# klebgenomics/Kaptive

Hardware: AMD Instinct MI355X
Metric: assemblies typed/sec (K+O) (higher is better)
Workload: dtype uint16x2 (exact; int32-equivalent); 1 GPU; 10000 synthetic 5 Mbp kpsc assemblies per GPU typed against the synthetic K-locus database, then the O-locus database; one step = all of them, as 10 batches of 1000 through context-owned work buffers; packed assemblies resident in HBM before the timed region; one alignment pass over the genes of both databases, one reduction per database; alignment_passes_per_batch=1, assemblies_per_gpu=10000, assemblies_total=10000, batch=1000, parallelism=1 x independent shard, no collective

## Files before the change

kaptive_amd/csrc/kp_align.hip:

```cpp
#include "kp_host.h"

static const char *const NO_RESULTS = "this batch has no resident alignment results (not aligned yet, or displaced: a context keeps the results of its KP_WORK_SLOTS most recently aligned batches)";

static int enqueue_forked(kp_ctx *ctx, kp_batch *b, KpWork *w, hipStream_t stream) {
    const KpAnchors an = w->anchors();
    const KpTasks tasks = w->tasks();
    const KpJoins joins = w->joins();
    const KpTrace trace = w->trace();
    kp_launch_join_chain(an, tasks, w->groups(), joins, w->d_jscratch.p, ctx->opt.join, w->jstream);
    kp_launch_join_fill(b->view, ctx->genes, joins, trace, ctx->opt.join, w->jstream);
    kp_launch_join_trace(b->view, ctx->genes, joins, tasks, trace, ctx->opt.join, w->jstream);
    kp_launch_task_order(b->view, ctx->genes, an, tasks, stream);
    KP_HIP_CHECK(ctx, hipEventRecord(w->ev[KP_EV_ORDER], stream));
    kp_launch_sw(b->view, ctx->genes, tasks, trace, ctx->max_gene_len > KP_FILL16_MAX_GENE_LEN, stream, w->ev[KP_EV_FILL]);
    KP_HIP_CHECK(ctx, hipEventRecord(w->ev[KP_EV_TRACEBACK], stream));
    return KP_OK;
}

static int enqueue_align(kp_ctx *ctx, kp_batch *b, KpWork *w) {
    const size_t n_asm = w->n_asm;
    for (auto &e : w->ev)
        if (!e) KP_HIP_CHECK(ctx, hipEventCreate(&e.h));
    if (!w->astream) KP_HIP_CHECK(ctx, hipStreamCreateWithFlags(&w->astream.h, hipStreamNonBlocking));
    if (!w->jstream) {
        KP_HIP_CHECK(ctx, hipStreamCreateWithFlags(&w->jstream.h, hipStreamNonBlocking));
        KP_HIP_CHECK(ctx, hipEventCreateWithFlags(&w->ev_jfork.h, hipEventDisableTiming));
        KP_HIP_CHECK(ctx, hipEventCreateWithFlags(&w->ev_jdone.h, hipEventDisableTiming));
    }
    hipStream_t stream = w->astream;
    const Event *ev = w->ev;
    if ((uint64_t)n_asm * w->anchor_cap > 0xFFFFFFF0ull)
        return kp_fail(ctx, KP_EOVERFLOW, "anchor buffer would exceed 2^32 entries; use smaller batches");
    if (((uint64_t)b->view.total_words << 4) >> KP_CAND_POS_BITS)
        return kp_fail(ctx, KP_EOVERFLOW, "a batch holds at most 2^33 bases (candidate positions); use smaller batches");
    KP_HIP_CHECK(ctx, w->d_anchors_a.reserve(n_asm * w->anchor_cap));
    KP_HIP_CHECK(ctx, w->d_anchors_b.reserve(n_asm * w->anchor_cap));
    KP_HIP_CHECK(ctx, w->d_counts.reserve(w->counts_len()));
    KP_HIP_CHECK(ctx, w->d_sub_counts.reserve(n_asm * KP_ANCHOR_SUBS));
    KP_HIP_CHECK(ctx, w->d_seg.reserve(w->seg_len()));
    KP_HIP_CHECK(ctx, w->d_tasks.reserve(KP_N_CLASSES * (size_t)w->task_cap));
    KP_HIP_CHECK(ctx, w->d_results.reserve(KP_N_CLASSES * (size_t)w->task_cap));
    KP_HIP_CHECK(ctx, w->d_task_drop.reserve(KP_N_CLASSES * (size_t)w->task_cap));
    KP_HIP_CHECK(ctx, w->d_jscratch.reserve(kp_join_chain_scratch_bytes(ctx->opt.join)));
    {
        uint32_t lg = 12;
        while (((uint64_t)1 << lg) < (uint64_t)b->max_asm_bases * 2 / 5 + 1 && lg < 31) ++lg;
        w->occ_log2 = lg;
        KP_HIP_CHECK(ctx, w->d_occ_keys.reserve((size_t)w->occ_slots << lg));
        KP_HIP_CHECK(ctx, w->d_occ_cnts.reserve((size_t)w->occ_slots << lg));
        KP_HIP_CHECK(ctx, w->d_occ_state.reserve(kp_occ_state_words(n_asm, w->occ_slots)));
    }
    KP_HIP_CHECK(ctx, w->d_task_order.reserve(w->order_len()));
    KP_HIP_CHECK(ctx, w->d_cand.reserve(w->cand_cap));
    KP_HIP_CHECK(ctx, w->d_cand_count.reserve(KP_CAND_COUNTS));
    KP_HIP_CHECK(ctx, w->d_ends.reserve(KP_N_CLASSES * (size_t)w->task_cap));
    KP_HIP_CHECK(ctx, w->d_trace_top.reserve(KP_TOP_WORDS));
    KP_HIP_CHECK(ctx, w->d_trace.reserve(w->trace_cap));
    KP_HIP_CHECK(ctx, w->d_groups.reserve(w->group_cap));
    KP_HIP_CHECK(ctx, w->d_joins.reserve(KP_N_CLASSES * (size_t)w->join_cap));
    KP_HIP_CHECK(ctx, w->d_join_counts.reserve(KP_JOIN_COUNTS));
    KP_HIP_CHECK(ctx, hipStreamWaitEvent(stream, b->in->ready, 0));
    if (b->after && b->after->in) KP_HIP_CHECK(ctx, hipStreamWaitEvent(stream, b->after->in->ready, 0));
    KP_HIP_CHECK(ctx, hipMemsetAsync(w->d_counts.p, 0, w->counts_len() * sizeof(uint32_t), stream));
    KP_HIP_CHECK(ctx, hipMemsetAsync(w->d_sub_counts.p, 0, n_asm * KP_ANCHOR_SUBS * sizeof(uint32_t), stream));
    KP_HIP_CHECK(ctx, hipMemsetAsync(w->d_cand_count.p, 0, KP_CAND_COUNTS * sizeof(unsigned long long), stream));
    KP_HIP_CHECK(ctx, hipMemsetAsync(w->d_task_order.p, 0, KP_ORDER_HEAD * sizeof(uint32_t), stream));
    KP_HIP_CHECK(ctx, hipMemsetAsync(w->d_trace_top.p, 0, KP_TOP_WORDS * sizeof(unsigned long long), stream));
    KP_HIP_CHECK(ctx, hipMemsetAsync(w->d_join_counts.p, 0, KP_JOIN_COUNTS * sizeof(uint32_t), stream));
    auto bits_for = [](uint64_t max_value) { uint32_t n = 1; while (n < 63 && (max_value >> n)) ++n; return n; };
    w->key_bits.qb = std::min<uint32_t>(16, bits_for((uint64_t)std::max(ctx->max_gene_len, 1)));
    w->key_bits.db = std::min<uint32_t>(30, bits_for((uint64_t)b->max_asm_bases + KP_DIAG_BIAS));
    const KpAnchors an = w->anchors();
    KP_HIP_CHECK(ctx, hipEventRecord(ev[KP_EV_START], stream));
    kp_launch_scan(b->view, ctx->index, w->d_cand.p, w->d_cand_count.p, w->cand_cap, an, ctx->opt.scan_mode, b->n_ctg_total, stream, ev[KP_EV_SCAN]);
    if (!ctx->opt.library_sort && kp_bsort_fits(2u * (uint32_t)ctx->n_genes)) {
        kp_launch_anchor_bsort(b->view, an, 2u * (uint32_t)ctx->n_genes, stream);
    } else {
        kp_launch_anchor_compact(b->view, an, stream);
        int rc = kp_sort_anchors(ctx, an, b->n_asm, &w->sort_temp.p, &w->sort_temp.bytes, w->seg_begin(), w->seg_end(),
                                 (int)(w->key_bits.qb + w->key_bits.db) + ctx->gs_bits, stream);
        if (rc) return rc;
    }
    KP_HIP_CHECK(ctx, hipEventRecord(ev[KP_EV_SORT], stream));
    kp_launch_occ_cut(b->view, ctx->d_gene_len.p, an, w->d_occ_keys.p, w->d_occ_cnts.p, w->d_occ_state.p, w->occ_demand(), w->occ_slots, w->occ_log2, stream);
    kp_launch_chain(b->view, an, w->tasks(), w->groups(), stream);
    KP_HIP_CHECK(ctx, hipMemsetAsync(w->d_task_drop.p, 0, KP_N_CLASSES * (size_t)w->task_cap, stream));
    KP_HIP_CHECK(ctx, hipEventRecord(w->ev_jfork, stream));
    KP_HIP_CHECK(ctx, hipStreamWaitEvent(w->jstream, w->ev_jfork, 0));
    const int rc = enqueue_forked(ctx, b, w, stream);
    const hipError_t e_done = hipEventRecord(w->ev_jdone, w->jstream), e_join = hipStreamWaitEvent(stream, w->ev_jdone, 0);
    if (rc) return rc;
    KP_HIP_CHECK(ctx, e_done);
    KP_HIP_CHECK(ctx, e_join);
    KP_HIP_CHECK(ctx, hipEventRecord(ev[KP_EV_JOINED], stream));
    KP_HIP_CHECK(ctx, hipEventRecord(ev[KP_EV_END], stream));
    KP_HIP_CHECK(ctx, hipGetLastError());
    return KP_OK;
}

static int sync_runs(kp_ctx *ctx, KpWork *w) {
    KP_HIP_CHECK(ctx, hipStreamSynchronize(ctx->post));
    for (auto &r : w->runs)
        if (r && r->stream) { KP_HIP_CHECK(ctx, hipStreamSynchronize(r->stream)); if (r->aux) KP_HIP_CHECK(ctx, hipStreamSynchronize(r->aux)); }
    return KP_OK;
}

KpWork *finalised_work(kp_ctx *ctx, kp_batch *b) {
    KpWork *w = work_of(b);
    if (!w) { kp_fail(ctx, KP_ESTATE, NO_RESULTS); return nullptr; }
    if (!w->finalised) { kp_fail(ctx, KP_ESTATE, "kp_batch_wait has not completed"); return nullptr; }
    return w;
}

extern "C" {

int kp_batch_align(kp_ctx *ctx, kp_batch *b) {
    if (!ctx || !b || b->ctx != ctx) return kp_fail(ctx, KP_EINVAL, "bad context/batch");
    if (!ctx->has_db) return kp_fail(ctx, KP_ESTATE, "no database loaded");
    KP_HIP_CHECK(ctx, hipSetDevice(ctx->device));
    KpWork *w = work_of(b);
    if (!w) {
        w = &ctx->work[ctx->next_slot++ % KP_WORK_SLOTS];
        if (w->owner) {
            if (int rc = sync_runs(ctx, w)) return rc;
            w->owner->w = nullptr;
        }
        w->owner = b; w->n_asm = (size_t)b->n_asm;
        b->w = w; b->last_w = w;
    }
    kp_caps_size(ctx->opt, ctx->learnt, b->n_asm, b->view.total_words, *w);
    w->aligned = false; w->finalised = false;
    w->cs_on = ctx->opt.cs != 0; w->cs_valid = false;
    w->cigar_on = ctx->opt.cigar != 0 || w->cs_on; w->cigar_valid = false;
    for (auto &v : w->h_tasks) v.clear();
    w->reset_runs();
    w->stats[KP_STAT_RERUNS] = 0;
    int rc = enqueue_align(ctx, b, w);
    if (rc) return rc;
    w->aligned = true;
    return KP_OK;
}

static int finalise_hits_on_device(kp_ctx *ctx, kp_batch *b, KpWork *w) {
    const size_t n_asm = w->n_asm;
    for (int attempt = 0;; ++attempt) {
        KP_HIP_CHECK(ctx, w->d_hits_raw.reserve(n_asm * w->hit_cap));
        KP_HIP_CHECK(ctx, w->d_hits.reserve(n_asm * w->hit_cap));
        KP_HIP_CHECK(ctx, w->d_keys.reserve(n_asm * w->hit_cap * 3));
        KP_HIP_CHECK(ctx, w->d_hit_counts.reserve(w->hit_counts_len()));
        KP_HIP_CHECK(ctx, w->d_cells.reserve(1));
        KP_HIP_CHECK(ctx, hipMemsetAsync(w->d_hit_counts.p, 0, w->hit_counts_len() * sizeof(uint32_t), ctx->post));
        KP_HIP_CHECK(ctx, hipMemsetAsync(w->d_cells.p, 0, sizeof(unsigned long long), ctx->post));
        kp_launch_hit_finalise(b->view, ctx->d_gene_len.p, w->tasks(), w->joins(), w->raw_hits(), w->hits(), w->d_cells.p, ctx->ln_half(), ctx->ln_int(), ctx->post);
        KP_HIP_CHECK(ctx, hipGetLastError());
        w->h_hit_counts.resize(w->hit_counts_len());
        unsigned long long cells = 0;
        if (int frc = fetch_all(ctx, ctx->post, {{w->h_hit_counts.data(), w->d_hit_counts.p, w->hit_counts_len() * sizeof(uint32_t)}, {&cells, w->d_cells.p, sizeof cells}}))
            return frc;
        const uint32_t max_raw = n_asm ? *std::max_element(w->h_raw_hit_count(), w->h_raw_hit_count() + n_asm) : 0;
        if (max_raw <= w->hit_cap) { w->stats[KP_STAT_CELLS] = (int64_t)cells; break; }
        if (attempt >= 2) return kp_fail(ctx, KP_EOVERFLOW, "hit buffers overflowed repeatedly");
        kp_caps_grow_hits(ctx->learnt, *w, max_raw, true);
        w->stats[KP_STAT_RERUNS] += 1;
    }
    w->hit_off.assign(n_asm + 1, 0);
    for (size_t a = 0; a < n_asm; ++a) w->hit_off[a + 1] = w->hit_off[a] + (int64_t)w->h_hit_count()[a];
    return KP_OK;
}

static int emit_cigars(kp_ctx *ctx, kp_batch *b, KpWork *w) {
    const size_t n_asm = w->n_asm;
    const int64_t total = w->hit_off[n_asm];
    w->cigar_cap = kp_caps_cigar_size(ctx->opt, ctx->learnt, (uint64_t)total);
    KP_HIP_CHECK(ctx, w->d_cig_src.reserve(n_asm * w->hit_cap));
    KP_HIP_CHECK(ctx, w->d_cig_cnt.reserve((size_t)total));
    KP_HIP_CHECK(ctx, w->d_cig_off.reserve((size_t)total + 1));
    KP_HIP_CHECK(ctx, w->d_cig_hit_off.reserve(n_asm + 1));
    KP_HIP_CHECK(ctx, w->d_cig_ops.reserve(w->cigar_cap));
    KP_HIP_CHECK(ctx, hipMemcpyAsync(w->d_cig_hit_off.p, w->hit_off.data(), (n_asm + 1) * sizeof(int64_t), hipMemcpyHostToDevice, ctx->post));
    kp_launch_cigar_locate(b->view, ctx->d_gene_len.p, w->tasks(), w->joins(), w->hits(), w->d_cig_src.p, ctx->post);
    kp_launch_cigar_walk(b->view, ctx->genes, w->tasks(), w->joins(), w->trace(), w->hits(), w->hit_rows(), w->d_cig_src.p, w->cigars(), false, ctx->post);
    for (int attempt = 0;; ++attempt) {
        kp_launch_cigar_walk(b->view, ctx->genes, w->tasks(), w->joins(), w->trace(), w->hits(), w->hit_rows(), w->d_cig_src.p, w->cigars(), true, ctx->post);
        KP_HIP_CHECK(ctx, hipGetLastError());
        int64_t need = 0;
        if (int frc = fetch_all(ctx, ctx->post, {{&need, w->d_cig_off.p + total, sizeof need}})) return frc;
        w->cigar_total = need;
        if (kp_caps_after_cigar(ctx->learnt, w->cigar_cap, (uint64_t)total, (uint64_t)need)) break;
        if (attempt >= 1) return kp_fail(ctx, KP_EOVERFLOW, "CIGAR buffer overflowed repeatedly");
        KP_HIP_CHECK(ctx, w->d_cig_ops.reserve(w->cigar_cap));
    }
    w->cigar_valid = true;
    return KP_OK;
}

static int emit_cs(kp_ctx *ctx, kp_batch *b, KpWork *w) {
    const int64_t total = w->hit_off[w->n_asm];
    w->cs_cap = kp_caps_cs_size(ctx->cs_caps, (uint64_t)total);
    KP_HIP_CHECK(ctx, w->d_cs_cnt.reserve((size_t)total));
    KP_HIP_CHECK(ctx, w->d_cs_off.reserve((size_t)total + 1));
    KP_HIP_CHECK(ctx, w->d_cs_bytes.reserve(w->cs_cap));
    kp_launch_cs_walk(b->view, ctx->genes, w->hits(), w->hit_rows(), w->cigars(), w->cs(), false, ctx->post);
    for (int attempt = 0;; ++attempt) {
        kp_launch_cs_walk(b->view, ctx->genes, w->hits(), w->hit_rows(), w->cigars(), w->cs(), true, ctx->post);
        KP_HIP_CHECK(ctx, hipGetLastError());
        int64_t need = 0;
        if (int frc = fetch_all(ctx, ctx->post, {{&need, w->d_cs_off.p + total, sizeof need}})) return frc;
        w->cs_total = need;
        if (kp_caps_after_cs(ctx->cs_caps, w->cs_cap, (uint64_t)total, (uint64_t)need)) break;
        if (attempt >= 1) return kp_fail(ctx, KP_EOVERFLOW, "cs buffer overflowed repeatedly");
        KP_HIP_CHECK(ctx, w->d_cs_bytes.reserve(w->cs_cap));
    }
    w->cs_valid = true;
    return KP_OK;
}

static const char *const NO_CS = "this batch has no cs strings (aligned without the cs option, or its hit table was replaced)";
static const char *const NO_CIGARS = "this batch has no CIGARs (aligned without the cigar option, or its hit table was replaced)";

int kp_batch_wait(kp_ctx *ctx, kp_batch *b) {
    if (!ctx || !b || b->ctx != ctx) return kp_fail(ctx, KP_EINVAL, "bad context/batch");
    KpWork *w = work_of(b);
    if (!w || !w->aligned) return kp_fail(ctx, KP_ESTATE, w ? "kp_batch_align has not been called" : NO_RESULTS);
    if (w->finalised) return KP_OK;
    KP_HIP_CHECK(ctx, hipSetDevice(ctx->device));
    const size_t n_asm = w->n_asm;
    const uint32_t *const n_join = w->h_join_count();
    for (;;) {
        KP_HIP_CHECK(ctx, hipStreamWaitEvent(ctx->post, w->ev[KP_EV_END], 0));
        w->h_counts.resize(w->counts_len());
        unsigned long long n_cand[KP_CAND_COUNTS] = {}, top[KP_TOP_WORDS] = {};
        if (int frc = fetch_all(ctx, ctx->post, {{w->h_counts.data(), w->d_counts.p, w->counts_len() * sizeof(uint32_t)},
                                                 {n_cand, w->d_cand_count.p, sizeof n_cand}, {top, w->d_trace_top.p, sizeof top},
                                                 {w->h_join_counts, w->d_join_counts.p, sizeof w->h_join_counts}}))
            return frc;
        KpPassSeen seen;
        seen.n_asm = n_asm; seen.total_words = b->view.total_words; seen.n_cand = n_cand[KP_CAND_FRONT] + n_cand[KP_CAND_BACK];
        seen.trace_need = top[KP_TOP_TRACE]; seen.occ_need = top[KP_TOP_OCC];
        seen.n_group = w->h_group_count();
        for (int c = 0; c < KP_N_CLASSES; ++c) seen.max_join = std::max(seen.max_join, n_join[c]);
        for (size_t a = 0; a < n_asm; ++a) seen.max_slice = std::max(seen.max_slice, w->h_slice_need()[a]);
        for (int c = 0; c < KP_N_CLASSES; ++c) seen.max_task = std::max(seen.max_task, w->h_task_count()[c]);
        if (ctx->opt.join_stats)
            std::fprintf(stderr, "[kp_batch_wait] %zu assemblies: %u groups, joins per band class %u %u %u %u, %llu assemblies needed their mid_occ (%u tables)\n", n_asm, seen.n_group,
                         n_join[0], n_join[1], n_join[2], n_join[3], (unsigned long long)seen.occ_need, w->occ_slots);
        std::string err;
        const KpCapsVerdict verdict = kp_caps_after_pass(ctx->learnt, *w, seen, err);
        if (verdict == KP_CAPS_FITTED) break;
        if (verdict == KP_CAPS_OVERFLOW) return kp_fail(ctx, KP_EOVERFLOW, err);
        w->stats[KP_STAT_RERUNS] += 1;
        int rc = enqueue_align(ctx, b, w);
        if (rc) return rc;
    }
    int64_t n_anchor = 0, n_task = 0;
    for (size_t a = 0; a < n_asm; ++a) n_anchor += w->h_anchor_count()[a];
    for (int c = 0; c < KP_N_CLASSES; ++c) n_task += w->h_task_count()[c];
    for (auto &v : w->h_tasks) v.clear();
    w->h_joins.clear();
    int rc = finalise_hits_on_device(ctx, b, w);
    if (rc) return rc;
    w->stats[KP_STAT_ANCHORS] = n_anchor; w->stats[KP_STAT_TASKS] = n_task; w->stats[KP_STAT_HITS] = w->hit_off[n_asm];
    if (w->cigar_on)
        if (int crc = emit_cigars(ctx, b, w)) return crc;
    if (w->cs_on)
        if (int crc = emit_cs(ctx, b, w)) return crc;
    w->finalised = true;
    return KP_OK;
}

int kp_batch_hit_offsets(kp_ctx *ctx, kp_batch *b, int64_t *hit_off) {
    if (!ctx || !b || b->ctx != ctx || !hit_off) return kp_fail(ctx, KP_EINVAL, "bad arguments");
    KpWork *w = finalised_work(ctx, b);
    if (!w) return KP_ESTATE;
    std::memcpy(hit_off, w->hit_off.data(), w->hit_off.size() * sizeof(int64_t));
    return KP_OK;
}

int kp_batch_hits(kp_ctx *ctx, kp_batch *b, kp_hit *out, int64_t cap) {
    if (!ctx || !b || b->ctx != ctx || (!out && cap > 0)) return kp_fail(ctx, KP_EINVAL, "bad arguments");
    KpWork *w = finalised_work(ctx, b);
    if (!w) return KP_ESTATE;
    const size_t n_asm = w->n_asm;
    const KpHitTable hits = w->hits();
    if (cap < w->hit_off[n_asm]) return kp_fail(ctx, KP_EINVAL, "hit buffer too small");
    KP_HIP_CHECK(ctx, hipSetDevice(ctx->device));
    for (size_t a = 0; a < n_asm; ++a) {
        const int64_t n = w->hit_off[a + 1] - w->hit_off[a];
        if (n > 0)
            KP_HIP_CHECK(ctx, hipMemcpyAsync(out + w->hit_off[a], hits.of(a), (size_t)n * sizeof(kp_hit), hipMemcpyDeviceToHost, ctx->post));
    }
    KP_HIP_CHECK(ctx, hipStreamSynchronize(ctx->post));
    return KP_OK;
}

int kp_batch_set_hits(kp_ctx *ctx, kp_batch *b, const kp_hit *hits, const int64_t *hit_off) {
    if (!ctx || !b || b->ctx != ctx || !hit_off) return kp_fail(ctx, KP_EINVAL, "bad arguments");
    KpWork *w = finalised_work(ctx, b);
    if (!w) return KP_ESTATE;
    const size_t n_asm = w->n_asm;
    int64_t max_n = 0;
    for (size_t a = 0; a < n_asm; ++a) {
        const int64_t n = hit_off[a + 1] - hit_off[a];
        if (n < 0 || (n > 0 && !hits)) return kp_fail(ctx, KP_EINVAL, "hit offsets must ascend");
        max_n = std::max(max_n, n);
    }
    if (max_n > (1 << 24)) return kp_fail(ctx, KP_EOVERFLOW, "too many hits for one assembly");
    KP_HIP_CHECK(ctx, hipSetDevice(ctx->device));
    if (int rc = sync_runs(ctx, w)) return rc;
    if ((uint64_t)max_n > w->hit_cap) kp_caps_grow_hits(ctx->learnt, *w, (uint32_t)max_n, false);
    KP_HIP_CHECK(ctx, w->d_hits.reserve(n_asm * w->hit_cap));
    KP_HIP_CHECK(ctx, w->d_hit_counts.reserve(w->hit_counts_len()));
    w->h_hit_counts.resize(w->hit_counts_len());
    const KpHitTable table = w->hits();
    w->hit_off.assign(n_asm + 1, 0);
    for (size_t a = 0; a < n_asm; ++a) {
        const int64_t n = hit_off[a + 1] - hit_off[a];
        if (n > 0)
            KP_HIP_CHECK(ctx, hipMemcpy(table.of(a), hits + hit_off[a], (size_t)n * sizeof(kp_hit), hipMemcpyHostToDevice));
        w->h_hit_count()[a] = (uint32_t)n;
        w->hit_off[a + 1] = w->hit_off[a] + n;
    }
    if (n_asm)
        KP_HIP_CHECK(ctx, hipMemcpy(table.count, w->h_hit_count(), n_asm * sizeof(uint32_t), hipMemcpyHostToDevice));
    w->stats[KP_STAT_HITS] = w->hit_off[n_asm];
    w->cigar_valid = false; w->cs_valid = false;
    w->reset_runs();
    return KP_OK;
}

int kp_batch_cigar_offsets(kp_ctx *ctx, kp_batch *b, int64_t *cigar_off) {
    if (!ctx || !b || b->ctx != ctx || !cigar_off) return kp_fail(ctx, KP_EINVAL, "bad arguments");
    KpWork *w = finalised_work(ctx, b);
    if (!w) return KP_ESTATE;
    if (!w->cigar_valid) return kp_fail(ctx, KP_ESTATE, NO_CIGARS);
    KP_HIP_CHECK(ctx, hipSetDevice(ctx->device));
    KP_HIP_CHECK(ctx, hipMemcpyAsync(cigar_off, w->d_cig_off.p, ((size_t)w->hit_off[(size_t)b->n_asm] + 1) * sizeof(int64_t), hipMemcpyDeviceToHost, ctx->post));
    KP_HIP_CHECK(ctx, hipStreamSynchronize(ctx->post));
    return KP_OK;
}

int kp_batch_cigars(kp_ctx *ctx, kp_batch *b, uint32_t *ops, int64_t cap) {
    if (!ctx || !b || b->ctx != ctx || (!ops && cap > 0)) return kp_fail(ctx, KP_EINVAL, "bad arguments");
    KpWork *w = finalised_work(ctx, b);
    if (!w) return KP_ESTATE;
    if (!w->cigar_valid) return kp_fail(ctx, KP_ESTATE, NO_CIGARS);
    if (cap < w->cigar_total) return kp_fail(ctx, KP_EINVAL, "CIGAR buffer too small");
    KP_HIP_CHECK(ctx, hipSetDevice(ctx->device));
    if (w->cigar_total > 0) {
        KP_HIP_CHECK(ctx, hipMemcpyAsync(ops, w->d_cig_ops.p, (size_t)w->cigar_total * sizeof(uint32_t), hipMemcpyDeviceToHost, ctx->post));
        KP_HIP_CHECK(ctx, hipStreamSynchronize(ctx->post));
    }
    return KP_OK;
}

int kp_batch_cs_offsets(kp_ctx *ctx, kp_batch *b, int64_t *cs_off) {
    if (!ctx || !b || b->ctx != ctx || !cs_off) return kp_fail(ctx, KP_EINVAL, "bad arguments");
    KpWork *w = finalised_work(ctx, b);
    if (!w) return KP_ESTATE;
    if (!w->cs_valid) return kp_fail(ctx, KP_ESTATE, NO_CS);
    KP_HIP_CHECK(ctx, hipSetDevice(ctx->device));
    KP_HIP_CHECK(ctx, hipMemcpyAsync(cs_off, w->d_cs_off.p, ((size_t)w->hit_off[(size_t)b->n_asm] + 1) * sizeof(int64_t), hipMemcpyDeviceToHost, ctx->post));
    KP_HIP_CHECK(ctx, hipStreamSynchronize(ctx->post));
    return KP_OK;
}

int kp_batch_cs(kp_ctx *ctx, kp_batch *b, char *bytes, int64_t cap) {
    if (!ctx || !b || b->ctx != ctx || (!bytes && cap > 0)) return kp_fail(ctx, KP_EINVAL, "bad arguments");
    KpWork *w = finalised_work(ctx, b);
    if (!w) return KP_ESTATE;
    if (!w->cs_valid) return kp_fail(ctx, KP_ESTATE, NO_CS);
    if (cap < w->cs_total) return kp_fail(ctx, KP_EINVAL, "cs buffer too small");
    KP_HIP_CHECK(ctx, hipSetDevice(ctx->device));
    if (w->cs_total > 0) {
        KP_HIP_CHECK(ctx, hipMemcpyAsync(bytes, w->d_cs_bytes.p, (size_t)w->cs_total, hipMemcpyDeviceToHost, ctx->post));
        KP_HIP_CHECK(ctx, hipStreamSynchronize(ctx->post));
    }
    return KP_OK;
}

int kp_batch_stats(kp_ctx *ctx, kp_batch *b, int64_t *stats5) {
    if (!ctx || !b || b->ctx != ctx || !stats5) return kp_fail(ctx, KP_EINVAL, "bad arguments");
    KpWork *w = finalised_work(ctx, b);
    if (!w) return KP_ESTATE;
    std::memcpy(stats5, w->stats, sizeof w->stats);
    return KP_OK;
}

int kp_batch_profile(kp_ctx *ctx, kp_batch *b, float *ms7, int64_t *bytes_scanned) {
    if (!ctx || !b || b->ctx != ctx || !ms7) return kp_fail(ctx, KP_EINVAL, "bad arguments");
    KpWork *w = finalised_work(ctx, b);
    if (!w) return KP_ESTATE;
    KP_HIP_CHECK(ctx, hipSetDevice(ctx->device));
    for (int i = KP_EV_START; i < KP_EV_END; ++i) {
        const KpPassEvent next = KpPassEvent(i + 1);
        if (hipEventElapsedTime(&ms7[i], w->ev[i], w->ev[next]) != hipSuccess) return kp_fail(ctx, KP_EHIP, "event timing failed");
    }
    if (bytes_scanned) *bytes_scanned = 4 * b->view.total_words;
    return KP_OK;
}

int64_t kp_batch_anchors(kp_ctx *ctx, kp_batch *b, int32_t a, uint64_t *out, int64_t cap) {
    if (!ctx || !b || b->ctx != ctx || a < 0 || a >= b->n_asm) return kp_fail(ctx, KP_EINVAL, "bad arguments");
    KpWork *w = finalised_work(ctx, b);
    if (!w) return KP_ESTATE;
    const int64_t n = w->h_anchor_count()[a];
    const int64_t m = std::min(n, cap);
    if (out && m > 0) {
        if (hipMemcpy(out, w->anchors().of((size_t)a), (size_t)m * sizeof(uint64_t), hipMemcpyDeviceToHost) != hipSuccess)
            return kp_fail(ctx, KP_EHIP, "D2H anchors failed");
        for (int64_t i = 0; i < m; ++i) out[i] = kp_key_unpack(out[i], w->key_bits);
    }
    return n;
}

int64_t kp_batch_tasks(kp_ctx *ctx, kp_batch *b, int32_t a, int32_t *out8, int64_t cap) {
    if (!ctx || !b || b->ctx != ctx || a < 0 || a >= b->n_asm) return kp_fail(ctx, KP_EINVAL, "bad arguments");
    KpWork *w = finalised_work(ctx, b);
    if (!w) return KP_ESTATE;
    for (int c = 0; c < KP_N_CLASSES; ++c) {
        const size_t nt = w->h_task_count()[c];
        if (w->h_tasks[c].size() == nt) continue;
        w->h_tasks[c].resize(nt);
        if (nt && hipMemcpy(w->h_tasks[c].data(), w->tasks().cls(c), nt * sizeof(KpTask), hipMemcpyDeviceToHost) != hipSuccess)
            return kp_fail(ctx, KP_EHIP, "D2H tasks failed");
    }
    int64_t n = 0;
    for (int c = 0; c < KP_N_CLASSES; ++c)
        for (const KpTask &t : w->h_tasks[c]) {
            if (t.asm_id != a || t.n_anchors == 0) continue;
            if (out8 && n < cap) {
                int32_t *o = out8 + 8 * n;
                o[0] = t.gs; o[1] = t.contig; o[2] = t.lo; o[3] = t.width; o[4] = t.n_anchors; o[5] = (int32_t)(t.qspan & 0xFFFFu); o[6] = (int32_t)(t.qspan >> 16); o[7] = t.chain_score;
            }
            ++n;
        }
    return n;
}

int64_t kp_batch_task_results(kp_ctx *ctx, kp_batch *b, int32_t a, int32_t *out7, int64_t cap) {
    if (!ctx || !b || b->ctx != ctx || a < 0 || a >= b->n_asm) return kp_fail(ctx, KP_EINVAL, "bad arguments");
    const int64_t n_tasks = kp_batch_tasks(ctx, b, a, nullptr, 0);
    if (n_tasks < 0) return n_tasks;
    KpWork *w = finalised_work(ctx, b);
    if (!w) return KP_ESTATE;
    int64_t n = 0;
    std::vector<KpSwResult> res;
    for (int c = 0; c < KP_N_CLASSES; ++c) {
        const size_t nt = w->h_tasks[c].size();
        res.resize(nt);
        if (nt && hipMemcpy(res.data(), w->tasks().cls_results(c), nt * sizeof(KpSwResult), hipMemcpyDeviceToHost) != hipSuccess)
            return kp_fail(ctx, KP_EHIP, "D2H task results failed");
        for (size_t i = 0; i < nt; ++i) {
            if (w->h_tasks[c][i].asm_id != a || w->h_tasks[c][i].n_anchors == 0) continue;
            if (out7 && n < cap) {
                const KpSwResult &r = res[i];
                int32_t *o = out7 + 7 * n;
                o[0] = r.score; o[1] = r.q_start; o[2] = r.q_end; o[3] = r.t_start; o[4] = r.t_end; o[5] = r.matches; o[6] = r.block_len;
            }
            ++n;
        }
    }
    return n;
}

int64_t kp_batch_joins(kp_ctx *ctx, kp_batch *b, int32_t a, int32_t *out, int64_t cap) {
    if (!ctx || !b || b->ctx != ctx || a < 0 || a >= b->n_asm) return kp_fail(ctx, KP_EINVAL, "bad arguments");
    KpWork *w = finalised_work(ctx, b);
    if (!w) return KP_ESTATE;
    size_t total = 0;
    for (int c = 0; c < KP_N_CLASSES; ++c) total += w->h_join_count()[c];
    if (w->h_joins.size() != total) {
        w->h_joins.resize(total);
        size_t at = 0;
        for (int c = 0; c < KP_N_CLASSES; ++c) {
            const size_t nj = w->h_join_count()[c];
            if (nj && hipMemcpy(w->h_joins.data() + at, w->joins().cls(c), nj * sizeof(KpJoin), hipMemcpyDeviceToHost) != hipSuccess)
                return kp_fail(ctx, KP_EHIP, "D2H joins failed");
            at += nj;
        }
    }
    int64_t n = 0;
    for (const KpJoin &J : w->h_joins) {
        if (J.asm_id != a) continue;
        if (out && n < cap) {
            int32_t *o = out + KP_JOIN_ROW_INTS * n;
            std::memset(o, 0, KP_JOIN_ROW_INTS * sizeof(int32_t));
            o[0] = J.gs; o[1] = J.contig; o[2] = J.n_pieces; o[3] = J.n_anchors; o[4] = J.chain_score; o[5] = J.width;
            for (int k = 0; k < J.n_pieces; ++k) {
                o[6 + k] = J.lo[k];
                int32_t *pr = o + 6 + KP_JOIN_MAX_PIECES + 11 * k;
                pr[0] = J.state[k]; pr[1] = J.visited[k];
                if (J.state[k] == 1) std::memcpy(pr + 2, J.res[k], 9 * sizeof(int32_t));
            }
        }
        ++n;
    }
    return n;
}

}
```

kaptive_amd/csrc/kp_cigar.hip:

```cpp
#include <algorithm>

#include "kp_hits.h"
#include "kp_internal.h"
#include "kp_reduce_core.h"
#include "kp_walk.h"

namespace {

constexpr unsigned long long SRC_NONE = ~0ull;
constexpr int LO_BIAS = 1 << 30;
constexpr int WALK_THREADS = 256;
constexpr int SCAN_THREADS = 1024;

__device__ __forceinline__ unsigned long long src_key(bool join, int lo, uint32_t ref) {
    return ((unsigned long long)(join ? 1u : 0u) << 63) | ((unsigned long long)(uint32_t)(lo + LO_BIAS) << 32) | ref;
}

__device__ __forceinline__ void claim(const kp_hit *h, int n, const kp_hit &mine, unsigned long long key, unsigned long long *src) {
    for (int i = kp_lower_bound_gene(h, n, mine.gene); i < n && h[i].gene == mine.gene; ++i) {
        if (!kp_same_span(h[i], mine)) continue;
        if (h[i].score == KP_HIT_SCORE(mine.score) && h[i].matches == mine.matches && h[i].block_len == mine.block_len && h[i].n_seeds == mine.n_seeds)
            atomicMin(&src[i], key);
        return;
    }
}

__global__ __launch_bounds__(256) void kp_cigar_locate_tasks_kernel(KpBatchView b, const int32_t *__restrict__ gene_len,
                                                                    const KpTask *__restrict__ tasks, const KpSwResult *__restrict__ results,
                                                                    const uint8_t *__restrict__ task_drop, const uint32_t *__restrict__ task_count,
                                                                    uint32_t task_cap, const kp_hit *__restrict__ hits,
                                                                    const uint32_t *__restrict__ n_hits, uint32_t hit_cap,
                                                                    unsigned long long *__restrict__ src) {
    const int cls = blockIdx.y;
    uint32_t n = task_count[cls];
    if (n > task_cap) n = task_cap;
    for (uint32_t i = blockIdx.x * blockDim.x + threadIdx.x; i < n; i += gridDim.x * blockDim.x) {
        const size_t at = (size_t)cls * task_cap + i;
        const KpTask t = tasks[at];
        kp_hit mine;
        if (!kp_task_hit(b, gene_len, t, results[at], task_drop[at] != 0, &mine)) continue;
        claim(hits + (size_t)t.asm_id * hit_cap, (int)min(n_hits[t.asm_id], hit_cap), mine, src_key(false, t.lo, KP_TASK_REF(cls, i)),
              src + (size_t)t.asm_id * hit_cap);
    }
}

__device__ __forceinline__ uint32_t join_ref(int cls, uint32_t ji, int k) { return ((uint32_t)cls << 28) | (ji << 3) | (uint32_t)k; }
static_assert(KP_JOIN_MAX_PIECES <= 8, "three bits of a join's reference name the piece");

__global__ __launch_bounds__(64) void kp_cigar_locate_joins_kernel(KpBatchView b, const int32_t *__restrict__ gene_len,
                                                                   const KpJoin *__restrict__ joins, const uint32_t *__restrict__ join_count,
                                                                   uint32_t join_cap, const kp_hit *__restrict__ hits,
                                                                   const uint32_t *__restrict__ n_hits, uint32_t hit_cap,
                                                                   unsigned long long *__restrict__ src) {
    const int cls = blockIdx.y;
    uint32_t n = join_count[cls];
    if (n > join_cap) n = join_cap;
    for (uint32_t i = blockIdx.x * blockDim.x + threadIdx.x; i < n; i += gridDim.x * blockDim.x) {
        const KpJoin &J = joins[(size_t)cls * join_cap + i];
        for (int k = 1; k < J.n_pieces; ++k) {
            kp_hit mine;
            if (!kp_join_piece_hit(b, gene_len, J, k, &mine)) continue;
            claim(hits + (size_t)J.asm_id * hit_cap, (int)min(n_hits[J.asm_id], hit_cap), mine, src_key(true, J.lo[k], join_ref(cls, i, k)),
                  src + (size_t)J.asm_id * hit_cap);
        }
    }
}

struct OpRuns {
    uint32_t *out;
    int64_t pos, cap;
    int op = -1;
    uint32_t len = 0, n = 0;
    __device__ __forceinline__ void flush() {
        if (op < 0) return;
        ++n;
        if (out) {
            --pos;
            if (pos >= 0 && pos < cap) out[pos] = (len << 4) | (uint32_t)op;
        }
    }
    __device__ __forceinline__ void run(int o, int k) {
        if (k <= 0) return;
        if (o == op) { len += (uint32_t)k; return; }
        flush();
        op = o; len = (uint32_t)k;
    }
};

template <bool EMIT>
__global__ __launch_bounds__(WALK_THREADS) void kp_cigar_walk_kernel(KpBatchView b, KpGenes genes, const KpTask *__restrict__ tasks,
                                                                     const KpSwEnd *__restrict__ ends, uint32_t task_cap,
                                                                     const KpJoin *__restrict__ joins, uint32_t join_cap,
                                                                     const uint4 *__restrict__ trace, const uint32_t *__restrict__ n_hits,
                                                                     uint32_t hit_cap, const int64_t *__restrict__ hit_off,
                                                                     const unsigned long long *__restrict__ src, uint32_t *__restrict__ cnt,
                                                                     const int64_t *__restrict__ off, uint32_t *__restrict__ ops, int64_t ops_cap) {
    for (int a = blockIdx.x; a < b.n_asm; a += gridDim.x) {
        const uint32_t n = min(n_hits[a], hit_cap);
        for (uint32_t i0 = 0; i0 < n; i0 += WALK_THREADS) {
            const uint32_t i = i0 + threadIdx.x;
            const bool have = i < n;
            const unsigned long long key = have ? src[(size_t)a * hit_cap + i] : SRC_NONE;
            const bool is_join = key != SRC_NONE && (key >> 63) != 0, is_task = key != SRC_NONE && !is_join;
            const uint32_t ref = (uint32_t)key;
            const int cls = is_task || is_join ? (int)(ref >> 28) : 0, P = 4 << cls;
            const int64_t row = hit_off[a] + i;
            OpRuns v;
            v.out = EMIT ? ops : nullptr; v.cap = ops_cap; v.pos = EMIT && have ? off[row + 1] : 0;
            KpTask tk;
            tk.asm_id = a; tk.gs = 0; tk.contig = 0; tk.lo = 0;
            KpSwEnd e;
            e.score = 0; e.er = 0; e.eb = 0; e.trace_off = 0;
            const KpJoin *J = joins + (size_t)cls * join_cap + (is_join ? (ref & 0x0FFFFFFFu) >> 3 : 0u);
            if (is_task) {
                const size_t at = (size_t)cls * task_cap + KP_REF_SLOT(ref);
                tk = tasks[at]; e = ends[at];
            }
            const KpTaskSeqs s = kp_task_seqs(b, genes, a, is_join ? J->gs : tk.gs, is_join ? J->contig : tk.contig);
            int q0 = 0, r_hi;
            if (is_task) kp_task_rows(tk.lo, 4 * P, s.t.cstart, s.t.cend, s.q.len, &q0, &r_hi);
            KpBandPath bp;
            kp_band_walk(is_task, tk.lo, P, q0, e.er, e.eb & 255, false, trace + e.trace_off, s, bp, v);
            if (is_join) {
                KpJoinPath jp;
                kp_join_walk(J, (int)(ref & 7u), P, s, trace, jp, v);
            }
            v.flush();
            if (!EMIT && have) cnt[row] = v.n;
        }
    }
}

__global__ __launch_bounds__(SCAN_THREADS) void kp_cigar_scan_kernel(const uint32_t *__restrict__ cnt, int64_t n, int64_t *__restrict__ off) {
    __shared__ int64_t s_sum[SCAN_THREADS];
    const int tid = threadIdx.x;
    const int64_t per = (n + SCAN_THREADS - 1) / SCAN_THREADS;
    const int64_t lo = (int64_t)tid * per < n ? (int64_t)tid * per : n, hi = lo + per < n ? lo + per : n;
    int64_t mine = 0;
    for (int64_t i = lo; i < hi; ++i) mine += cnt[i];
    s_sum[tid] = mine;
    __syncthreads();
    for (int o = 1; o < SCAN_THREADS; o <<= 1) {
        const int64_t v = tid >= o ? s_sum[tid - o] : 0;
        __syncthreads();
        s_sum[tid] += v;
        __syncthreads();
    }
    int64_t at = s_sum[tid] - mine;
    for (int64_t i = lo; i < hi; ++i) { off[i] = at; at += cnt[i]; }
    if (tid == SCAN_THREADS - 1) off[n] = s_sum[tid];
}

}

void kp_launch_cigar_locate(const KpBatchView &b, const int32_t *gene_len, const KpTasks &t, const KpJoins &j, const KpHitTable &hits,
                            unsigned long long *src, hipStream_t stream) {
    (void)hipMemsetAsync(src, 0xFF, (size_t)b.n_asm * hits.cap * sizeof(unsigned long long), stream);
    hipLaunchKernelGGL(kp_cigar_locate_tasks_kernel, dim3(256, KP_N_CLASSES), dim3(256), 0, stream, b, gene_len, t.tasks, t.results, t.drop, t.count,
                       t.cap, hits.rows, hits.count, hits.cap, src);
    hipLaunchKernelGGL(kp_cigar_locate_joins_kernel, dim3(16, KP_N_CLASSES), dim3(64), 0, stream, b, gene_len, j.list, j.count, j.cap, hits.rows,
                       hits.count, hits.cap, src);
}

void kp_launch_count_scan(const uint32_t *cnt, int64_t n, int64_t *off, hipStream_t stream) {
    hipLaunchKernelGGL(kp_cigar_scan_kernel, dim3(1), dim3(SCAN_THREADS), 0, stream, cnt, n, off);
}

void kp_launch_cigar_walk(const KpBatchView &b, const KpGenes &genes, const KpTasks &t, const KpJoins &j, const KpTrace &trace, const KpHitTable &hits,
                          const KpHitRows &rows, const unsigned long long *src, const KpPerHit<uint32_t> &cig, bool emit, hipStream_t stream) {
    const dim3 grid((unsigned)std::min(std::max(b.n_asm, 1), 4096)), block(WALK_THREADS);
    if (!emit) {
        hipLaunchKernelGGL(kp_cigar_walk_kernel<false>, grid, block, 0, stream, b, genes, t.tasks, t.ends, t.cap, j.list, j.cap, trace.units, hits.count,
                           hits.cap, rows.hit_off, src, cig.cnt, (const int64_t *)nullptr, (uint32_t *)nullptr, (int64_t)0);
        return kp_launch_count_scan(cig.cnt, rows.total, cig.off, stream);
    }
    hipLaunchKernelGGL(kp_cigar_walk_kernel<true>, grid, block, 0, stream, b, genes, t.tasks, t.ends, t.cap, j.list, j.cap, trace.units, hits.count,
                       hits.cap, rows.hit_off, src, (uint32_t *)nullptr, cig.off, cig.data, cig.cap);
}
```

kaptive_amd/csrc/kp_ctx.hip:

```cpp
#include <cctype>
#include <cstdlib>
#include <mutex>
#include <new>
#include <unordered_map>
#include <sys/mman.h>

#include "kp_host.h"

static std::mutex g_err_mutex;
static std::string g_global_error = "";

std::atomic<long long> g_dev_allocs{0};
bool g_debug_alloc = false;

static std::mutex g_pin_mutex;
struct PinBlock { size_t bytes; bool mapped, locked; };
static std::unordered_map<void *, PinBlock> g_pin_blocks;
static size_t g_pin_bytes = 0;
constexpr size_t HUGE_PAGE = (size_t)2 << 20;
hipError_t pinned_alloc(void **out, size_t bytes) {
    const hipError_t e = hipHostMalloc(out, bytes, hipHostMallocPortable);
    if (e == hipSuccess) {
        std::lock_guard<std::mutex> lk(g_pin_mutex);
        g_pin_blocks[*out] = PinBlock{bytes, false, true};
        g_pin_bytes += bytes;
    }
    return e;
}
static void *mapped_alloc(size_t bytes) {
    bytes = (bytes + HUGE_PAGE - 1) & ~(HUGE_PAGE - 1);
    char *raw = (char *)mmap(nullptr, bytes + HUGE_PAGE, PROT_READ | PROT_WRITE, MAP_PRIVATE | MAP_ANONYMOUS, -1, 0);
    if (raw == MAP_FAILED) return nullptr;
    char *p = (char *)(((uintptr_t)raw + HUGE_PAGE - 1) & ~(uintptr_t)(HUGE_PAGE - 1));
    if (p > raw) munmap(raw, (size_t)(p - raw));
    if (raw + HUGE_PAGE > p) munmap(p + bytes, (size_t)(raw + HUGE_PAGE - p));
    (void)madvise(p, bytes, MADV_HUGEPAGE);
    std::lock_guard<std::mutex> lk(g_pin_mutex);
    g_pin_blocks[p] = PinBlock{bytes, true, false};
    return p;
}
static hipError_t mapped_lock(void *p) {
    size_t bytes;
    {
        std::lock_guard<std::mutex> lk(g_pin_mutex);
        auto it = g_pin_blocks.find(p);
        if (it == g_pin_blocks.end() || !it->second.mapped) return hipErrorInvalidValue;
        if (it->second.locked) return hipSuccess;
        bytes = it->second.bytes;
    }
    const hipError_t e = hipHostRegister(p, bytes, hipHostRegisterPortable);
    if (e == hipSuccess) {
        std::lock_guard<std::mutex> lk(g_pin_mutex);
        g_pin_blocks[p].locked = true;
        g_pin_bytes += bytes;
    }
    return e;
}
void pinned_free(void *p) {
    if (!p) return;
    PinBlock b{0, false, true};
    {
        std::lock_guard<std::mutex> lk(g_pin_mutex);
        auto it = g_pin_blocks.find(p);
        if (it != g_pin_blocks.end()) {
            b = it->second;
            if (b.locked) g_pin_bytes -= b.bytes;
            g_pin_blocks.erase(it);
        }
    }
    if (b.mapped) {
        if (b.locked) (void)hipHostUnregister(p);
        munmap(p, b.bytes);
    } else {
        (void)hipHostFree(p);
    }
}

int kp_fail(kp_ctx *ctx, int code, const std::string &msg) {
    if (ctx) ctx->error = msg;
    else {
        std::lock_guard<std::mutex> lk(g_err_mutex);
        g_global_error = msg;
    }
    return code;
}

hipError_t create_priority_stream(hipStream_t *stream) {
    int least = 0, greatest = 0;
    hipError_t e = hipDeviceGetStreamPriorityRange(&least, &greatest);
    if (e != hipSuccess) return e;
    return hipStreamCreateWithPriority(stream, hipStreamDefault, greatest);
}

static uint32_t env_u32(const char *name, uint32_t dflt) {
    const char *v = std::getenv(name);
    if (!v || !*v) return dflt;
    const long long x = std::atoll(v);
    return x > 0 ? (uint32_t)x : dflt;
}

static void options_from_env(KpOptions &o) {
    o.anchor_cap = env_u32("KAPTIVE_AMD_ANCHOR_CAP", o.anchor_cap);
    o.tasks_per_asm = env_u32("KAPTIVE_AMD_TASKS_PER_ASM", o.tasks_per_asm);
    o.hit_cap = env_u32("KAPTIVE_AMD_HIT_CAP", o.hit_cap);
    o.trace_kb_per_asm = env_u32("KAPTIVE_AMD_TRACE_KB_PER_ASM", o.trace_kb_per_asm);
    o.trace_set = env_u32("KAPTIVE_AMD_TRACE_KB_PER_ASM", 0) != 0;
    o.cand_cap = env_u32("KAPTIVE_AMD_CAND_CAP", 0);
    o.group_cap = env_u32("KAPTIVE_AMD_GROUP_CAP", o.group_cap);
    o.join_cap = env_u32("KAPTIVE_AMD_JOIN_CAP", o.join_cap);
    o.occ_slots = env_u32("KAPTIVE_AMD_OCC_SLOTS", o.occ_slots);
    o.kept_cap = env_u32("KAPTIVE_AMD_KEPT_CAP", o.kept_cap);
    o.piece_cap = env_u32("KAPTIVE_AMD_PIECE_CAP", o.piece_cap);
    o.prot_cap = env_u32("KAPTIVE_AMD_PROT_CAP", o.prot_cap);
    o.scan_mode = (int)env_u32("KAPTIVE_AMD_SCAN_ABLATE", 0);
    o.library_sort = (int)env_u32("KAPTIVE_AMD_LIBRARY_SORT", 0);
    o.upload_piece_mb = std::max<uint32_t>(1, env_u32("KAPTIVE_AMD_UPLOAD_PIECE_MB", 4096));
    { const char *rb = getenv("KAPTIVE_AMD_READBACK"); o.readback_copy_engine = rb && std::string(rb) == "copy"; }
    o.spin_wait = (int)env_u32("KAPTIVE_AMD_SPIN_WAIT", 0);
    o.join_stats = std::getenv("KAPTIVE_AMD_JOIN_STATS") != nullptr;
    if (const char *e = std::getenv("KAPTIVE_AMD_JOIN_GRID")) std::sscanf(e, "%d,%d,%d,%d", &o.join.fill, &o.join.walk, &o.join.chain, &o.join.chain_large);
    if (const char *e = std::getenv("KAPTIVE_AMD_JOIN_PRIO")) o.join.prio = std::atoi(e);
    if (const char *e = std::getenv("KAPTIVE_AMD_SKIP_JOINS")) o.join.skip = std::atoi(e);
    g_debug_alloc = std::getenv("KAPTIVE_AMD_DEBUG_ALLOC") != nullptr;
}

static void fill_blosum(int8_t *m) {
    static const int8_t b[25][25] = {
        {4, -1, -2, -2, 0, -1, -1, 0, -2, -1, -1, -1, -1, -2, -1, 1, 0, -3, -2, 0, -2, -1, -1, -1, -4},
        {-1, 5, 0, -2, -3, 1, 0, -2, 0, -3, -2, 2, -1, -3, -2, -1, -1, -3, -2, -3, -1, -2, 0, -1, -4},
        {-2, 0, 6, 1, -3, 0, 0, 0, 1, -3, -3, 0, -2, -3, -2, 1, 0, -4, -2, -3, 4, -3, 0, -1, -4},
        {-2, -2, 1, 6, -3, 0, 2, -1, -1, -3, -4, -1, -3, -3, -1, 0, -1, -4, -3, -3, 4, -3, 1, -1, -4},
        {0, -3, -3, -3, 9, -3, -4, -3, -3, -1, -1, -3, -1, -2, -3, -1, -1, -2, -2, -1, -3, -1, -3, -1, -4},
        {-1, 1, 0, 0, -3, 5, 2, -2, 0, -3, -2, 1, 0, -3, -1, 0, -1, -2, -1, -2, 0, -2, 4, -1, -4},
        {-1, 0, 0, 2, -4, 2, 5, -2, 0, -3, -3, 1, -2, -3, -1, 0, -1, -3, -2, -2, 1, -3, 4, -1, -4},
        {0, -2, 0, -1, -3, -2, -2, 6, -2, -4, -4, -2, -3, -3, -2, 0, -2, -2, -3, -3, -1, -4, -2, -1, -4},
        {-2, 0, 1, -1, -3, 0, 0, -2, 8, -3, -3, -1, -2, -1, -2, -1, -2, -2, 2, -3, 0, -3, 0, -1, -4},
        {-1, -3, -3, -3, -1, -3, -3, -4, -3, 4, 2, -3, 1, 0, -3, -2, -1, -3, -1, 3, -3, 3, -3, -1, -4},
        {-1, -2, -3, -4, -1, -2, -3, -4, -3, 2, 4, -2, 2, 0, -3, -2, -1, -2, -1, 1, -4, 3, -3, -1, -4},
        {-1, 2, 0, -1, -3, 1, 1, -2, -1, -3, -2, 5, -1, -3, -1, 0, -1, -3, -2, -2, 0, -3, 1, -1, -4},
        {-1, -1, -2, -3, -1, 0, -2, -3, -2, 1, 2, -1, 5, 0, -2, -1, -1, -1, -1, 1, -3, 2, -1, -1, -4},
        {-2, -3, -3, -3, -2, -3, -3, -3, -1, 0, 0, -3, 0, 6, -4, -2, -2, 1, 3, -1, -3, 0, -3, -1, -4},
        {-1, -2, -2, -1, -3, -1, -1, -2, -2, -3, -3, -1, -2, -4, 7, -1, -1, -4, -3, -2, -2, -3, -1, -1, -4},
        {1, -1, 1, 0, -1, 0, 0, 0, -1, -2, -2, 0, -1, -2, -1, 4, 1, -3, -2, -2, 0, -2, 0, -1, -4},
        {0, -1, 0, -1, -1, -1, -1, -2, -2, -1, -1, -1, -1, -2, -1, 1, 5, -2, -2, 0, -1, -1, -1, -1, -4},
        {-3, -3, -4, -4, -2, -2, -3, -2, -2, -3, -2, -3, -1, 1, -4, -3, -2, 11, 2, -3, -4, -2, -2, -1, -4},
        {-2, -2, -2, -3, -2, -1, -2, -3, 2, -1, -1, -2, -1, 3, -3, -2, -2, 2, 7, -1, -3, -1, -2, -1, -4},
        {0, -3, -3, -3, -1, -2, -2, -3, -3, 3, 1, -2, 1, -1, -2, -2, 0, -3, -1, 4, -3, 2, -2, -1, -4},
        {-2, -1, 4, 4, -3, 0, 1, -1, 0, -3, -4, 0, -3, -3, -2, 0, -1, -4, -3, -3, 4, -3, 0, -1, -4},
        {-1, -2, -3, -3, -1, -2, -3, -4, -3, 3, 3, -3, 2, 0, -3, -2, -1, -2, -1, 2, -3, 3, -3, -1, -4},
        {-1, 0, 0, 1, -3, 4, 4, -2, 0, -3, -3, 1, -1, -3, -1, 0, -1, -2, -2, -2, 0, -3, 4, -1, -4},
        {-1, -1, -1, -1, -1, -1, -1, -1, -1, -1, -1, -1, -1, -1, -1, -1, -1, -1, -1, -1, -1, -1, -1, -1, -4},
        {-4, -4, -4, -4, -4, -4, -4, -4, -4, -4, -4, -4, -4, -4, -4, -4, -4, -4, -4, -4, -4, -4, -4, -4, 1},
    };
    static const char alphabet[] = "ARNDCQEGHILKMFPSTWYVBJZX*";
    std::memset(m, KP_PROT_FILL, 256 * 256);
    for (int x = 0; x < 25; ++x)
        for (int y = 0; y < 25; ++y) m[(uint8_t)alphabet[x] * 256 + (uint8_t)alphabet[y]] = b[x][y];
}

extern "C" {

int kp_device_count(void) {
    int n_dev = 0;
    const hipError_t e = hipGetDeviceCount(&n_dev);
    if (e != hipSuccess) return kp_fail(nullptr, KP_EHIP, std::string("hipGetDeviceCount: ") + hipGetErrorString(e));
    return n_dev;
}

int kp_device_numa_node(int device_id) {
    char bus[64] = {0};
    if (hipDeviceGetPCIBusId(bus, (int)sizeof bus, device_id) != hipSuccess) return -1;
    for (char *c = bus; *c; ++c) *c = (char)std::tolower((unsigned char)*c);
    const std::string path = std::string("/sys/bus/pci/devices/") + bus + "/numa_node";
    std::FILE *f = std::fopen(path.c_str(), "r");
    if (!f) return -1;
    int node = -1;
    if (std::fscanf(f, "%d", &node) != 1) node = -1;
    std::fclose(f);
    return node;
}

int kp_ctx_create(int device_id, kp_ctx **out) {
    if (!out) return kp_fail(nullptr, KP_EINVAL, "out is null");
    *out = nullptr;
    int n_dev = 0;
    hipError_t e = hipGetDeviceCount(&n_dev);
    if (e != hipSuccess || n_dev == 0)
        return kp_fail(nullptr, KP_EHIP, std::string("no HIP device available: ") + hipGetErrorString(e));
    if (device_id < 0 || device_id >= n_dev) return kp_fail(nullptr, KP_EINVAL, "device_id out of range");
    kp_ctx *ctx = new (std::nothrow) kp_ctx();
    if (!ctx) return kp_fail(nullptr, KP_ENOMEM, "out of host memory");
    ctx->device = device_id;
    options_from_env(ctx->opt);
    if ((e = hipSetDevice(device_id)) == hipSuccess && !ctx->opt.spin_wait) (void)hipSetDeviceFlags(hipDeviceScheduleBlockingSync);
    if (e != hipSuccess || (e = hipStreamCreate(&ctx->stream.h)) != hipSuccess || (e = hipStreamCreateWithFlags(&ctx->copy.h, hipStreamNonBlocking)) != hipSuccess ||
        (e = create_priority_stream(&ctx->post.h)) != hipSuccess || (e = create_priority_stream(&ctx->aux.h)) != hipSuccess) {
        delete ctx;
        return kp_fail(nullptr, KP_EHIP, std::string("device setup failed: ") + hipGetErrorString(e));
    }
    std::vector<int8_t> m(256 * 256);
    fill_blosum(m.data());
    std::vector<float> ln(KP_MAPQ_LN_HALF_SIZE + KP_MAPQ_LN_INT_SIZE, 0.0f);
    for (int i = 1; i < KP_MAPQ_LN_HALF_SIZE; ++i) ln[(size_t)i] = kp_mapq_ln((double)i / 2.0);
    for (int i = 1; i < KP_MAPQ_LN_INT_SIZE; ++i) ln[(size_t)KP_MAPQ_LN_HALF_SIZE + i] = kp_mapq_ln((double)i);
    if (upload(ctx, ctx->d_blosum, m.data(), m.size()) != KP_OK || upload(ctx, ctx->d_ln, ln.data(), ln.size()) != KP_OK || hipStreamSynchronize(ctx->stream) != hipSuccess) {
        std::string msg = ctx->error;
        kp_ctx_destroy(ctx);
        return kp_fail(nullptr, KP_EHIP, "substitution table upload failed: " + msg);
    }
    *out = ctx;
    return KP_OK;
}

void kp_ctx_destroy(kp_ctx *ctx) {
    if (!ctx) return;
    (void)hipSetDevice(ctx->device);
    (void)hipDeviceSynchronize();
    for (kp_batch *b : ctx->batches) {
        b->in.reset();
        b->ctx = nullptr; b->w = nullptr; b->last_w = nullptr;
    }
    delete ctx;
}

const char *kp_last_error(const kp_ctx *ctx) {
    if (ctx) return ctx->error.c_str();
    std::lock_guard<std::mutex> lk(g_err_mutex);
    static thread_local std::string copy;
    copy = g_global_error;
    return copy.c_str();
}

void *kp_ctx_stream(kp_ctx *ctx) { return ctx ? (void *)ctx->stream.h : nullptr; }

int kp_ctx_set_option(kp_ctx *ctx, const char *name, int64_t value) {
    if (!ctx) return kp_fail(nullptr, KP_EINVAL, "null context");
    if (!name || value < 0) return kp_fail(ctx, KP_EINVAL, "bad option");
    const std::string n(name);
    KpOptions &o = ctx->opt;
    if (kp_caps_set_option(o, ctx->learnt, ctx->run_caps, n, value)) return KP_OK;
    if (kp_caps_set_cs_option(ctx->cs_caps, n, value)) return KP_OK;
    if (n == "scan_mode") o.scan_mode = (int)value;
    else if (n == "library_sort") o.library_sort = value != 0;
    else if (n == "cigar") o.cigar = value != 0;
    else if (n == "cs") o.cs = value != 0;
    else if (n == "upload_piece_mb") o.upload_piece_mb = (uint32_t)std::max<int64_t>(1, std::min<int64_t>(value, 4096));
    else return kp_fail(ctx, KP_EINVAL, "unknown option: " + n);
    return KP_OK;
}

int kp_host_alloc(size_t bytes, void **out) {
    if (!out) return kp_fail(nullptr, KP_EINVAL, "out is null");
    *out = nullptr;
    if (bytes >= 4 * HUGE_PAGE) {
        int rc = kp_host_reserve(bytes, out);
        if (rc == KP_OK && (rc = kp_host_lock(*out)) == KP_OK) return KP_OK;
        if (*out) { pinned_free(*out); *out = nullptr; }
    }
    const hipError_t e = pinned_alloc(out, std::max<size_t>(bytes, 1));
    if (e != hipSuccess) return kp_fail(nullptr, KP_ENOMEM, std::string("hipHostMalloc: ") + hipGetErrorString(e));
    return KP_OK;
}

int kp_host_reserve(size_t bytes, void **out) {
    if (!out) return kp_fail(nullptr, KP_EINVAL, "out is null");
    *out = mapped_alloc(std::max<size_t>(bytes, 1));
    if (!*out) return kp_fail(nullptr, KP_ENOMEM, "mmap failed");
    return KP_OK;
}

int kp_host_lock(void *p) {
    const hipError_t e = mapped_lock(p);
    if (e == hipErrorInvalidValue) return kp_fail(nullptr, KP_EINVAL, "not a block of kp_host_reserve");
    if (e != hipSuccess) return kp_fail(nullptr, KP_ENOMEM, std::string("hipHostRegister: ") + hipGetErrorString(e));
    return KP_OK;
}

void kp_host_free(void *p) { pinned_free(p); }

int64_t kp_device_allocations(void) { return (int64_t)g_dev_allocs.load(std::memory_order_relaxed); }

int64_t kp_host_pinned_bytes(void) {
    std::lock_guard<std::mutex> lk(g_pin_mutex);
    return (int64_t)g_pin_bytes;
}

}
```

kaptive_amd/csrc/kp_host.h:

```cpp
#pragma once

#include <cstring>
#include <memory>
#include "kp_internal.h"
#include "kp_caps.h"
#include "kp_device.h"
#include "kp_reduce_core.h"
static_assert(KP_CAPS_ANCHOR_SUBS == KP_ANCHOR_SUBS, "the policy sizes the scan's sub-slices");

struct KpTypingGroup {
    int32_t gene_lo = 0, gene_hi = 0;
    DevBuf<uint16_t> d_gene_locus, d_gene_pos;
    DevBuf<uint8_t> d_gene_extra, d_prot_db;
    DevBuf<int8_t> d_gene_strand;
    DevBuf<int32_t> d_locus_off, d_locus_len, d_prot_db_off, d_prot_db_len;
    KpTypingDb typing{};
    int max_db_prot_len = 0;
};

struct KpTypingRun {
    hipStream_t stream = nullptr, aux = nullptr;
    Event ev_fork, ev_join;
    bool split = false;
    KpHitTable hits{};
    DevBuf<kp_hit> d_hits;
    DevBuf<uint32_t> d_hit_n;
    DevBuf<uint64_t> d_keys;
    DevBuf<uint32_t> d_order;
    DevBuf<uint8_t> d_flag;
    DevBuf<int32_t> d_dp_scratch;
    int kept_cap = 0, piece_cap = 0, prot_cap = 0;
    size_t n_asm = 0;
    DevBuf<uint32_t> d_pack;
    DevBuf<uint8_t> d_prot;
    DevBuf<double> d_scores;
    DevBuf<int32_t> d_lcounts, d_best, d_pairs, d_dp;
    DevBuf<KpKept> d_kept;
    DevBuf<KpPiece> d_pieces;
    DevBuf<KpAsmSummary> d_summary;
    KpTypingParams prm{};
    bool scored = false, reduced = false;
    bool sums_valid = false;
    std::vector<KpAsmSummary> h_sums;
    int32_t max_kept = 1, max_pieces = 1;
    size_t slots() const { return n_asm * (size_t)kept_cap; }
    size_t pairs_len() const { return 4 * slots() + n_asm + 1; }
    KpReduceTables tables() const {
        int32_t *const q = d_pairs.p, *const base = q + 4 * slots();
        return {.best = d_best.p, .keys = d_keys.p, .order = d_order.p, .kept_flag = d_flag.p, .kept = d_kept.p, .kept_cap = kept_cap,
                .pieces = d_pieces.p, .piece_cap = piece_cap, .summary = d_summary.p, .prot = d_prot.p, .prot_cap = prot_cap,
                .q_off = q, .q_len = q + slots(), .t_off = q + 2 * slots(), .t_len = q + 3 * slots(), .pair_base = base, .n_pairs = base + n_asm, .dp8 = d_dp.p};
    }
};

struct kp_batch;

struct KpOptions : KpCapOptions {
    int scan_mode = 0;
    int library_sort = 0;
    uint32_t upload_piece_mb = 4096;
    int readback_copy_engine = 0;
    int spin_wait = 0;
    int cigar = 0;
    int cs = 0;
    bool join_stats = false;
    KpJoinLaunch join;
};

struct KpInput {
    DevBuf<uint32_t> d_words;
    DevBuf<int64_t> d_asm_word_off;
    DevBuf<int32_t> d_ctg_start, d_ctg_len, d_asm_first_ctg, d_n_runs, d_asm_first_nrun;
    PinnedBlock h_stage;
    Event ready;
};

enum KpPassEvent { KP_EV_START, KP_EV_SCAN, KP_EV_SORT, KP_EV_ORDER, KP_EV_FILL, KP_EV_TRACEBACK, KP_EV_JOINED, KP_EV_END, KP_N_EVENTS };
static_assert(KP_EV_END == 7, "kp_batch_profile returns seven stage times");
enum KpStat { KP_STAT_ANCHORS, KP_STAT_TASKS, KP_STAT_CELLS, KP_STAT_HITS, KP_STAT_RERUNS, KP_N_STATS };
enum KpTopWord { KP_TOP_TRACE = 0, KP_TOP_OCC = 3, KP_TOP_WORDS = 4 };
enum KpJoinCount { KP_JOIN_GROUPS = 0, KP_JOIN_CLASSES = 1, KP_JOIN_COUNTS = 1 + KP_N_CLASSES };
enum KpCandCount { KP_CAND_FRONT, KP_CAND_BACK, KP_CAND_COUNTS };

struct KpWork : KpPassCaps {
    kp_batch *owner = nullptr;
    size_t n_asm = 0;
    KpKeyBits key_bits{16, 30};
    DevBuf<uint64_t> d_anchors_a, d_anchors_b;
    DevBuf<uint32_t> d_counts;
    size_t task_count_at() const { return n_asm; }
    size_t slice_need_at() const { return n_asm + KP_N_CLASSES; }
    size_t counts_len() const { return slice_need_at() + n_asm; }
    const uint32_t *h_anchor_count() const { return h_counts.data(); }
    const uint32_t *h_task_count() const { return h_counts.data() + task_count_at(); }
    const uint32_t *h_slice_need() const { return h_counts.data() + slice_need_at(); }
    DevBuf<uint32_t> d_sub_counts;
    DevBuf<uint64_t> d_cand;
    DevBuf<unsigned long long> d_cand_count;
    DevBuf<uint32_t> d_seg;
    size_t seg_len() const { return 2 * n_asm; }
    uint32_t *seg_begin() const { return d_seg.p; }
    uint32_t *seg_end() const { return d_seg.p + n_asm; }
    DevBuf<KpTask> d_tasks;
    DevBuf<KpSwResult> d_results;
    DevBuf<uint8_t> d_task_drop, d_jscratch;
    DevBuf<uint32_t> d_occ_keys, d_occ_cnts, d_occ_state;
    uint32_t occ_log2 = 0;
    DevBuf<KpSwEnd> d_ends;
    DevBuf<unsigned long long> d_trace_top;
    unsigned long long *occ_demand() const { return d_trace_top.p + KP_TOP_OCC; }
    Stream astream;
    Stream jstream;
    Event ev_jfork, ev_jdone;
    DevBuf<uint4> d_trace;
    DevBlock sort_temp;
    DevBuf<uint32_t> d_task_order;
    size_t order_len() const { return KP_ORDER_HEAD + KP_N_CLASSES * (size_t)task_cap; }
    DevBuf<KpGroup> d_groups;
    DevBuf<KpJoin> d_joins;
    DevBuf<uint32_t> d_join_counts;
    uint32_t h_join_counts[KP_JOIN_COUNTS] = {};
    uint32_t h_group_count() const { return h_join_counts[KP_JOIN_GROUPS]; }
    const uint32_t *h_join_count() const { return h_join_counts + KP_JOIN_CLASSES; }
    std::vector<KpJoin> h_joins;
    DevBuf<kp_hit> d_hits_raw, d_hits;
    DevBuf<uint32_t> d_hit_counts;
    size_t hit_counts_len() const { return 2 * n_asm; }
    uint32_t *h_raw_hit_count() { return h_hit_counts.data(); }
    uint32_t *h_hit_count() { return h_hit_counts.data() + n_asm; }
    DevBuf<uint64_t> d_keys;
    DevBuf<unsigned long long> d_cells;
    bool cigar_on = false, cigar_valid = false;
    uint64_t cigar_cap = 0;
    int64_t cigar_total = 0;
    DevBuf<unsigned long long> d_cig_src;
    DevBuf<uint32_t> d_cig_cnt, d_cig_ops;
    DevBuf<int64_t> d_cig_off, d_cig_hit_off;
    bool cs_on = false, cs_valid = false;
    uint64_t cs_cap = 0;
    int64_t cs_total = 0;
    DevBuf<uint32_t> d_cs_cnt;
    DevBuf<int64_t> d_cs_off;
    DevBuf<char> d_cs_bytes;
    std::vector<std::unique_ptr<KpTypingRun>> runs;
    bool aligned = false, finalised = false;
    std::vector<uint32_t> h_counts, h_hit_counts;
    std::vector<KpTask> h_tasks[KP_N_CLASSES];
    std::vector<int64_t> hit_off;
    int64_t stats[KP_N_STATS] = {};
    Event ev[KP_N_EVENTS];
    KpAnchors anchors() const {
        return {.keys = d_anchors_a.p, .count = d_counts.p, .cap = anchor_cap, .kb = key_bits, .sub_count = d_sub_counts.p,
                .sub_cap = anchor_cap / KP_ANCHOR_SUBS, .second = d_anchors_b.p, .need = d_counts.p + slice_need_at()};
    }
    KpTasks tasks() const {
        return {.tasks = d_tasks.p, .count = d_counts.p + task_count_at(), .cap = task_cap, .results = d_results.p, .ends = d_ends.p, .drop = d_task_drop.p,
                .order_head = d_task_order.p, .order_count = d_task_order.p + KP_ORDER_COUNTS, .order = d_task_order.p + KP_ORDER_HEAD};
    }
    KpGroups groups() const { return {.list = d_groups.p, .count = d_join_counts.p + KP_JOIN_GROUPS, .cap = group_cap}; }
    KpJoins joins() const { return {.list = d_joins.p, .count = d_join_counts.p + KP_JOIN_CLASSES, .cap = join_cap}; }
    KpTrace trace() const { return {.units = d_trace.p, .top = d_trace_top.p + KP_TOP_TRACE, .cap = trace_cap}; }
    KpHitTable raw_hits() const { return {.rows = d_hits_raw.p, .count = d_hit_counts.p, .cap = hit_cap, .keys = d_keys.p}; }
    KpHitTable hits() const { return {.rows = d_hits.p, .count = d_hit_counts.p + n_asm, .cap = hit_cap, .keys = nullptr}; }
    KpHitRows hit_rows() const { return {.hit_off = d_cig_hit_off.p, .total = hit_off[n_asm]}; }
    KpPerHit<uint32_t> cigars() const { return {.cnt = d_cig_cnt.p, .off = d_cig_off.p, .data = d_cig_ops.p, .cap = (int64_t)cigar_cap}; }
    KpPerHit<char> cs() const { return {.cnt = d_cs_cnt.p, .off = d_cs_off.p, .data = d_cs_bytes.p, .cap = (int64_t)cs_cap}; }
    void reset_runs() { for (auto &r : runs) if (r) r->split = r->scored = r->reduced = r->sums_valid = false; }
};

#define KP_INPUT_POOL 16

struct kp_ctx {
    int device = 0;
    PinnedBlock bounce;
    int gs_bits = 18;
    int max_gene_len = 0;
    Stream stream;
    Stream post;
    Stream aux;
    Stream copy;
    std::string error;
    KpOptions opt;
    KpLearnt learnt;
    KpCsCaps cs_caps;
    bool has_db = false;
    int32_t n_genes = 0;
    int64_t n_postings = 0;
    std::vector<int32_t> gene_len;
    DevBuf<uint2> d_slots;
    DevBuf<uint64_t> d_filter, d_filter2;
    DevBuf<uint64_t> d_postings;
    DevBuf<uint32_t> d_nib;
    DevBuf<int32_t> d_nib_off, d_gene_len;
    DevBuf<uint4> d_gene_prof;
    DevBuf<uint8_t> d_gene_has_n;
    KpSeedIndex index{};
    KpGenes genes{};
    DevBuf<int8_t> d_blosum;
    DevBuf<float> d_ln;
    const float *ln_half() const { return d_ln.p; }
    const float *ln_int() const { return d_ln.p + KP_MAPQ_LN_HALF_SIZE; }
    DevBuf<uint8_t> d_pq, d_pt;
    DevBuf<int32_t> d_pmeta, d_pout, d_pscratch;
    std::vector<std::unique_ptr<KpTypingGroup>> groups;
    std::vector<KpRunCaps> run_caps;
    struct GroupStreams { Stream stream, aux; };
    std::vector<GroupStreams> group_streams;
    KpWork work[KP_WORK_SLOTS];
    uint32_t next_slot = 0;
    std::vector<std::unique_ptr<KpInput>> free_inputs;
    std::vector<kp_batch *> batches;
};

struct kp_batch {
    kp_ctx *ctx = nullptr;
    int32_t n_asm = 0;
    std::unique_ptr<KpInput> in;
    const uint32_t *d_words = nullptr;
    KpBatchView view{};
    int64_t max_asm_bases = 0;
    int32_t n_ctg_total = 0;
    KpWork *w = nullptr;
    KpWork *last_w = nullptr;
    kp_batch *after = nullptr;
    int32_t group = 0;
};

hipError_t create_priority_stream(hipStream_t *stream);

struct Fetch {
    kp_ctx *ctx;
    hipStream_t stream;
    struct Item { void *dst; size_t off, bytes; };
    std::vector<Item> items;
    size_t used = 0;
    bool by_copy_engine;
    Fetch(kp_ctx *c, hipStream_t s) : ctx(c), stream(s), by_copy_engine(c->opt.readback_copy_engine != 0) {}
    ~Fetch() { if (!items.empty()) (void)hipStreamSynchronize(stream); }
    int begin(size_t total) {
        if (by_copy_engine) return KP_OK;
        total += 64 * 8;
        KP_HIP_CHECK(ctx, ctx->bounce.reserve(total, total + total / 4 + (1u << 20)));
        return KP_OK;
    }
    int add(void *dst, const void *src, size_t bytes) {
        if (!bytes) return KP_OK;
        if (by_copy_engine || (bytes & 3u)) { KP_HIP_CHECK(ctx, hipMemcpyAsync(dst, src, bytes, hipMemcpyDeviceToHost, stream)); return KP_OK; }
        if (used + bytes > ctx->bounce.bytes) return kp_fail(ctx, KP_ESTATE, "read-back larger than announced");
        kp_launch_read_back(src, ctx->bounce.p + used, bytes, stream);
        items.push_back(Item{dst, used, bytes});
        used = (used + bytes + 63) & ~(size_t)63;
        return KP_OK;
    }
    int finish() {
        const hipError_t e = hipStreamSynchronize(stream);
        if (e != hipSuccess) { items.clear(); used = 0; }
        KP_HIP_CHECK(ctx, e);
        for (const Item &it : items) std::memcpy(it.dst, ctx->bounce.p + it.off, it.bytes);
        items.clear(); used = 0;
        return KP_OK;
    }
};

struct FetchItem { void *dst; const void *src; size_t bytes; };
inline int fetch_all(kp_ctx *ctx, hipStream_t stream, std::initializer_list<FetchItem> items) {
    size_t total = 0;
    for (const FetchItem &i : items) total += i.bytes;
    Fetch f(ctx, stream);
    int rc = f.begin(total);
    for (const FetchItem &i : items) if (!rc) rc = f.add(i.dst, i.src, i.bytes);
    return rc ? rc : f.finish();
}

template <class T>
int upload(kp_ctx *ctx, DevBuf<T> &buf, const T *src, size_t n, hipStream_t stream = nullptr) {
    KP_HIP_CHECK(ctx, buf.reserve(n));
    if (n) KP_HIP_CHECK(ctx, hipMemcpyAsync(buf.p, src, n * sizeof(T), hipMemcpyHostToDevice, stream ? stream : ctx->stream.h));
    return KP_OK;
}

inline KpWork *work_of(kp_batch *b) {
    return (b->w && b->w->owner == b) ? b->w : nullptr;
}
KpWork *finalised_work(kp_ctx *ctx, kp_batch *b);
```

kaptive_amd/csrc/kp_internal.h:

```cpp
#pragma once

#include <hip/hip_runtime.h>
#include <stdint.h>

#include <string>
#include <vector>

#include "../../include/kaptive_amd.h"

#define KP_FILTER_LOG2 24
__host__ __device__ inline uint32_t kp_filter_block(uint32_t x) { return x & ((1u << (KP_FILTER_LOG2 - 6)) - 1u); }
__host__ __device__ inline uint2 kp_filter_mask2(uint32_t x) {
    uint2 m;
    m.x = 1u << ((x >> 18) & 31u);
    m.y = 1u << ((x >> 23) & 31u);
    return m;
}
__host__ __device__ inline bool kp_filter_test(uint2 got, uint32_t x) {
    return ((got.x >> ((x >> 18) & 31u)) & (got.y >> ((x >> 23) & 31u)) & 1u) != 0u;
}
__host__ __device__ inline uint64_t kp_filter_mask(uint32_t kmer) {
    const uint2 m = kp_filter_mask2(kmer);
    return ((uint64_t)m.y << 32) | m.x;
}
#define KP_FILTER2_LOG2 23
__host__ __device__ inline uint32_t kp_filter2_block(uint32_t kmer) { return (kmer * 0xC2B2AE35u) >> (32 - (KP_FILTER2_LOG2 - 6)); }
__host__ __device__ inline uint2 kp_filter2_mask2(uint32_t kmer) {
    const uint32_t h = kmer * 0x27D4EB2Fu;
    uint2 m;
    m.x = (1u << (h >> 27)) | (1u << ((h >> 22) & 31u));
    m.y = (1u << ((h >> 17) & 31u)) | (1u << ((h >> 12) & 31u));
    return m;
}
#define KP_CAND_POS_BITS 33
__host__ __device__ inline uint64_t kp_cand_pack(uint64_t pos, uint32_t z, uint32_t x) { return (pos << 31) | ((uint64_t)z << 30) | x; }
__host__ __device__ inline bool kp_seed_is_interior(int64_t t, int64_t S, int64_t E) { return t >= S + KP_W && t + KP_K + KP_W <= E; }

struct KpSeedIndex {
    const uint64_t *filter;
    const uint64_t *filter2;
    const uint2 *slots;
    const uint64_t *postings;
    uint32_t slot_mask;
    uint32_t slot_shift;
};

struct KpGenes {
    const uint32_t *nib;
    const int32_t *word_off;
    const int32_t *len;
    int32_t n_genes;
    const uint4 *prof;
    const uint8_t *has_n;
};

__host__ __device__ inline uint32_t kp_row_profile(uint32_t qcode) {
    return qcode < 4u ? ((6u << (3u * qcode)) | (3u << 12)) : (3u | (3u << 3) | (3u << 6) | (3u << 9) | (3u << 12));
}

struct KpKeyBits {
    uint32_t qb, db;
};
__host__ __device__ inline uint64_t kp_key_pack(uint64_t spec_key, KpKeyBits kb) {
    return ((spec_key >> 46) << (kb.qb + kb.db)) | (((spec_key >> 16) & 0x3FFFFFFFull) << kb.qb) | (spec_key & 0xFFFFull);
}
__host__ __device__ inline uint32_t kp_ckey_qpos(uint64_t k, KpKeyBits kb) { return (uint32_t)(k & ((1ull << kb.qb) - 1ull)); }
__host__ __device__ inline uint32_t kp_ckey_diag(uint64_t k, KpKeyBits kb) {
    return (uint32_t)((k >> kb.qb) & ((1ull << kb.db) - 1ull));
}
__host__ __device__ inline uint32_t kp_ckey_gs(uint64_t k, KpKeyBits kb) { return (uint32_t)(k >> (kb.qb + kb.db)); }
__host__ __device__ inline uint64_t kp_key_unpack(uint64_t k, KpKeyBits kb) {
    return ((uint64_t)kp_ckey_gs(k, kb) << 46) | ((uint64_t)kp_ckey_diag(k, kb) << 16) | kp_ckey_qpos(k, kb);
}

struct KpBatchView {
    const uint32_t *words;
    const int64_t *asm_word_off;
    const int32_t *ctg_start;
    const int32_t *ctg_len;
    const int32_t *asm_first_ctg;
    const int32_t *n_runs;
    const int32_t *asm_first_nrun;
    int32_t n_asm;
    int64_t total_words;
};

#define KP_N_CLASSES 4
struct KpTask {
    int32_t asm_id;
    int32_t gs;
    int32_t contig;
    int32_t lo;
    int32_t width;
    int32_t n_anchors;
    uint32_t qspan;
    int32_t chain_score;
};
static_assert(sizeof(KpTask) == 32, "KpTask is read as two 16-byte halves");

struct KpSwResult {
    int32_t score, q_start, q_end, t_start, t_end, matches, block_len;
};

__host__ __device__ inline void kp_task_rows(int lo, int width, int cstart, int cend, int qlen, int *r_lo, int *r_hi);
__host__ __device__ inline void kp_piece_rows(int lo, int width, int cstart, int cend, int qlen, int r0, int r1, int *r_lo, int *r_hi) {
    kp_task_rows(lo, width, cstart, cend, qlen, r_lo, r_hi);
    if (*r_lo < r0) *r_lo = r0;
    if (*r_hi > r1) *r_hi = r1;
    if (*r_hi < *r_lo) *r_hi = *r_lo;
}
__host__ __device__ inline void kp_task_rows(int lo, int width, int cstart, int cend, int qlen, int *r_lo, int *r_hi) {
    int a = cstart - lo - (width - 1);
    if (a < 0) a = 0;
    a &= ~7;
    int z = cend - lo;
    if (z > qlen) z = qlen;
    if (z < a) z = a;
    *r_lo = a;
    *r_hi = z;
}

struct KpSwEnd {
    int32_t score;
    int32_t er, eb;
    uint32_t trace_off;
};
#define KP_SWEND_HAS_N 0x100

#define KP_TASK_REF(cls, slot) (((uint32_t)(cls) << 28) | (uint32_t)(slot))
#define KP_REF_CLS(ref) ((ref) >> 28)
#define KP_REF_SLOT(ref) ((ref) & 0x0FFFFFFFu)
#define KP_REF_NONE 0xFFFFFFFFu
struct KpGroup {
    int32_t asm_id, n;
    int32_t gs, contig;
    uint32_t total;
    uint32_t task[KP_JOIN_GROUP_MAX];
    uint32_t first[KP_JOIN_GROUP_MAX];
    uint32_t cnt[KP_JOIN_GROUP_MAX];
};
struct KpJoin {
    int32_t asm_id, gs, contig, n_pieces, n_anchors, chain_score, width;
    int32_t lo[KP_JOIN_MAX_PIECES];
    int32_t cmask[KP_JOIN_MAX_PIECES];
    int32_t r0[KP_JOIN_MAX_PIECES], r1[KP_JOIN_MAX_PIECES];
    int32_t n_members;
    int32_t weak_mask;
    uint32_t member_task[KP_JOIN_GROUP_MAX];
    uint32_t trace_off[KP_JOIN_MAX_PIECES], export_off[KP_JOIN_MAX_PIECES];
    int32_t end_s[KP_JOIN_MAX_PIECES], end_r[KP_JOIN_MAX_PIECES], end_b[KP_JOIN_MAX_PIECES];
    int32_t state[KP_JOIN_MAX_PIECES], visited[KP_JOIN_MAX_PIECES];
    int32_t res[KP_JOIN_MAX_PIECES][9];
    int32_t drop_mask;
};

#define KP_HIP_CHECK(ctx, expr)                                                                     \
    do {                                                                                            \
        hipError_t e_ = (expr);                                                                     \
        if (e_ != hipSuccess) return kp_fail((ctx), KP_EHIP, std::string(#expr) + ": " + hipGetErrorString(e_)); \
    } while (0)

struct kp_ctx;
int kp_fail(kp_ctx *ctx, int code, const std::string &msg);

struct KpAnchors {
    uint64_t *keys;
    uint32_t *count;
    uint32_t cap;
    KpKeyBits kb;
    uint32_t *sub_count;
    uint32_t sub_cap;
    uint64_t *second;
    uint32_t *need;
    uint64_t *of(size_t a) const { return keys + a * cap; }
};
struct KpTasks {
    KpTask *tasks;
    uint32_t *count;
    uint32_t cap;
    KpSwResult *results;
    KpSwEnd *ends;
    uint8_t *drop;
    uint32_t *order_head, *order_count, *order;
    KpTask *cls(int c) const { return tasks + (size_t)c * cap; }
    KpSwResult *cls_results(int c) const { return results + (size_t)c * cap; }
};
struct KpGroups { KpGroup *list; uint32_t *count; uint32_t cap; };
struct KpJoins { KpJoin *list; uint32_t *count ; uint32_t cap; KpJoin *cls(int c) const { return list + (size_t)c * cap; } };
struct KpTrace { uint4 *units; unsigned long long *top; uint64_t cap; };
struct KpHitTable {
    kp_hit *rows;
    uint32_t *count;
    uint32_t cap;
    uint64_t *keys;
    kp_hit *of(size_t a) const { return rows + a * cap; }
};
struct KpHitRows { const int64_t *hit_off; int64_t total; };
template <class T>
struct KpPerHit { uint32_t *cnt; int64_t *off; T *data; int64_t cap; };
struct KpReduceTables {
    const int32_t *best;
    uint64_t *keys;
    uint32_t *order;
    uint8_t *kept_flag;
    kp_kept *kept; int kept_cap;
    kp_piece *pieces; int piece_cap;
    kp_asm_summary *summary;
    uint8_t *prot; int prot_cap;
    int32_t *q_off, *q_len, *t_off, *t_len, *pair_base, *n_pairs;
    int32_t *dp8;
};
struct KpJoinLaunch { int fill = 2048, walk = 512, chain = 2560, chain_large = 512, prio = 1, skip = 0; };

#define KP_ANCHOR_SUBS 64
void kp_launch_scan(const KpBatchView &b, const KpSeedIndex &idx, uint64_t *cand, unsigned long long *n_cand, uint64_t cand_cap,
                    const KpAnchors &an, int ablate_mode, int32_t n_ctg_total, hipStream_t stream, hipEvent_t after_scan);
void kp_launch_anchor_compact(const KpBatchView &b, const KpAnchors &an, hipStream_t stream);
size_t kp_occ_state_words(size_t n_asm, uint32_t occ_slots);
void kp_launch_occ_cut(const KpBatchView &b, const int32_t *gene_len, const KpAnchors &an, uint32_t *occ_keys, uint32_t *occ_cnts,
                       uint32_t *occ_state, unsigned long long *occ_demand, uint32_t occ_slots, uint32_t occ_log2_size, hipStream_t stream);
void kp_launch_chain(const KpBatchView &b, const KpAnchors &an, const KpTasks &tasks, const KpGroups &groups, hipStream_t stream);
void kp_launch_sw(const KpBatchView &b, const KpGenes &genes, const KpTasks &tasks, const KpTrace &trace, bool has_long_genes, hipStream_t stream, hipEvent_t after_fill);
#define KP_ORDER_BUCKETS 65
#define KP_ORDER_COUNTS (2 * KP_N_CLASSES * KP_ORDER_BUCKETS)
#define KP_ORDER_HEAD (KP_ORDER_COUNTS + 2 * KP_N_CLASSES)
void kp_launch_task_order(const KpBatchView &b, const KpGenes &genes, const KpAnchors &an, const KpTasks &tasks, hipStream_t stream);
void kp_launch_join_chain(const KpAnchors &an, const KpTasks &tasks, const KpGroups &groups, const KpJoins &joins, uint8_t *scratch,
                          const KpJoinLaunch &L, hipStream_t stream);
size_t kp_join_chain_scratch_bytes(const KpJoinLaunch &L);
void kp_launch_join_fill(const KpBatchView &b, const KpGenes &genes, const KpJoins &joins, const KpTrace &trace, const KpJoinLaunch &L, hipStream_t stream);
void kp_launch_join_trace(const KpBatchView &b, const KpGenes &genes, const KpJoins &joins, const KpTasks &tasks, const KpTrace &trace,
                          const KpJoinLaunch &L, hipStream_t stream);
void kp_launch_cigar_locate(const KpBatchView &b, const int32_t *gene_len, const KpTasks &tasks, const KpJoins &joins, const KpHitTable &hits,
                            unsigned long long *src, hipStream_t stream);
void kp_launch_cigar_walk(const KpBatchView &b, const KpGenes &genes, const KpTasks &tasks, const KpJoins &joins, const KpTrace &trace, const KpHitTable &hits,
                          const KpHitRows &rows, const unsigned long long *src, const KpPerHit<uint32_t> &cig, bool emit, hipStream_t stream);
void kp_launch_count_scan(const uint32_t *cnt, int64_t n, int64_t *off, hipStream_t stream);
void kp_launch_cs_walk(const KpBatchView &b, const KpGenes &genes, const KpHitTable &hits, const KpHitRows &rows, const KpPerHit<uint32_t> &cig,
                       const KpPerHit<char> &cs, bool emit, hipStream_t stream);
void kp_launch_hit_split(const KpHitTable &hits, int32_t gene_lo, int32_t gene_hi, const KpHitTable &out, int32_t n_asm, hipStream_t stream);
struct KpTypingDb;
void kp_launch_hit_finalise(const KpBatchView &b, const int32_t *gene_len, const KpTasks &tasks, const KpJoins &joins, const KpHitTable &raw,
                            const KpHitTable &hits, unsigned long long *cells, const float *ln_half, const float *ln_int, hipStream_t stream);
void kp_launch_score(const KpBatchView &b, const KpHitTable &hits, const KpTypingDb &db, double min_cov, double *scores, int32_t *counts, hipStream_t stream);
void kp_launch_reduce(const KpBatchView &b, const KpHitTable &hits, const KpTypingDb &db, const kp_typing_params &prm, const KpReduceTables &t, hipStream_t stream);
void kp_launch_states(const KpBatchView &b, const KpTypingDb &db, const kp_typing_params &prm, const KpReduceTables &t, hipStream_t stream);
void kp_launch_read_back(const void *src, void *dst_pinned, size_t bytes, hipStream_t stream);
void kp_launch_pack_rows(const uint32_t *src, size_t src_pitch, uint32_t *dst, size_t dst_pitch, size_t width, int rows,
                         hipStream_t stream);
#define KP_PROT_ROWBUF_FIELDS 8
void kp_launch_protein(const uint8_t *q, const int32_t *q_off, const int32_t *q_len, const uint8_t *t,
                       const int32_t *t_off, const int32_t *t_len, int32_t n, const int32_t *n_dev, const int8_t *blosum,
                       int32_t *out8, int32_t *scratch, size_t scratch_ints_per_block, int n_blocks, hipStream_t stream,
                       hipStream_t aux, hipEvent_t fork, hipEvent_t join,
                       const int32_t *seed_off = nullptr, int seed_k = 0);
bool kp_bsort_fits(uint32_t n_bins);
void kp_launch_anchor_bsort(const KpBatchView &b, const KpAnchors &an, uint32_t n_bins, hipStream_t stream);
int kp_sort_anchors(kp_ctx *ctx, const KpAnchors &an, int32_t n_asm, void **temp, size_t *temp_bytes, uint32_t *d_seg_begin,
                    uint32_t *d_seg_end, int end_bit, hipStream_t stream);
```

kaptive_amd/csrc/kp_sw.hip:

```cpp
#include "kp_internal.h"
#include "kp_walk.h"

namespace {

constexpr int CH = 64;
constexpr int TG = KP_TRACE_GROUP;
constexpr int OE = KP_GAP_OPEN + KP_GAP_EXT;
constexpr int EX = KP_GAP_EXT;
static_assert(KP_SC_MATCH == 2 && KP_SC_MISMATCH == -4 && KP_SC_N == -1 && OE == 6 && EX == 2,
              "the profile fields and the biases below encode these scores");
static_assert(2 * KP_FILL16_MAX_GENE_LEN + 14 < 0x7C00, "biased scores must stay below the half-precision infinity pattern (pk_max3) "
                                                 "and leave bit 15 of a half-word free for the guard");

constexpr unsigned K1 = 0x00010001u;
constexpr unsigned GUARD = 0x80008000u;
constexpr unsigned CB = 12;
constexpr unsigned ZB = CB - OE;
constexpr unsigned GAP_NONE = (CB - OE - EX) * K1;
constexpr unsigned GAP_EDGE = (CB - OE) * K1;
constexpr unsigned T_OUT = 12u;
constexpr unsigned PROF_OUT = 0u;

template <bool ROW>
__device__ __forceinline__ unsigned from_lower(unsigned v) {
    return (unsigned)(ROW ? __builtin_amdgcn_mov_dpp((int)v, 0x111 , 0xf, 0xf, true)
                          : __builtin_amdgcn_mov_dpp((int)v, 0x138 , 0xf, 0xf, true));
}
template <bool ROW>
__device__ __forceinline__ unsigned from_upper(unsigned v) {
    return (unsigned)(ROW ? __builtin_amdgcn_mov_dpp((int)v, 0x101 , 0xf, 0xf, true)
                          : __builtin_amdgcn_mov_dpp((int)v, 0x130 , 0xf, 0xf, true));
}


template <unsigned LIT>
__device__ __forceinline__ unsigned add_k(unsigned a) {
    unsigned r;
    asm("v_add_u32_e32 %0, %2, %1" : "=v"(r) : "v"(a), "n"(LIT));
    return r;
}
template <unsigned LIT>
__device__ __forceinline__ unsigned or_k(unsigned a) {
    unsigned r;
    asm("v_or_b32_e32 %0, %2, %1" : "=v"(r) : "v"(a), "n"(LIT));
    return r;
}
template <unsigned LIT>
__device__ __forceinline__ unsigned and_k(unsigned a) {
    unsigned r;
    asm("v_and_b32_e32 %0, %2, %1" : "=v"(r) : "v"(a), "n"(LIT));
    return r;
}
__device__ __forceinline__ unsigned add_v(unsigned a, unsigned b) {
    unsigned r;
    asm("v_add_u32_e32 %0, %1, %2" : "=v"(r) : "v"(a), "v"(b));
    return r;
}
__device__ __forceinline__ unsigned sub_v(unsigned a, unsigned b) {
    unsigned r;
    asm("v_sub_u32_e32 %0, %1, %2" : "=v"(r) : "v"(a), "v"(b));
    return r;
}
__device__ __forceinline__ unsigned or_v(unsigned a, unsigned b) {
    unsigned r;
    asm("v_or_b32_e32 %0, %1, %2" : "=v"(r) : "v"(a), "v"(b));
    return r;
}
template <int N>
__device__ __forceinline__ unsigned shr_k(unsigned a) {
    unsigned r;
    asm("v_lshrrev_b32_e32 %0, %2, %1" : "=v"(r) : "v"(a), "n"(N));
    return r;
}
__device__ __forceinline__ unsigned pk_max(unsigned a, unsigned b) {
    unsigned r;
    asm("v_pk_max_u16 %0, %1, %2" : "=v"(r) : "v"(a), "v"(b));
    return r;
}
__device__ __forceinline__ unsigned pk_max3(unsigned a, unsigned b, unsigned c) {
    unsigned r;
#ifdef KP_SW_NO_MAX3
    asm("v_pk_max_u16 %0, %1, %2" : "=v"(r) : "v"(a), "v"(b));
    asm("v_pk_max_u16 %0, %1, %2" : "=v"(r) : "v"(r), "v"(c));
#else
    asm("v_pk_maximum3_f16 %0, %1, %2, %3" : "=v"(r) : "v"(a), "v"(b), "v"(c));
#endif
    return r;
}
__device__ __forceinline__ unsigned pk_shr(unsigned v, unsigned by) {
    unsigned r;
    asm("v_pk_lshrrev_b16 %0, %1, %2" : "=v"(r) : "v"(by), "v"(v));
    return r;
}
__device__ __forceinline__ unsigned pk_sign_mask(unsigned v, unsigned fifteen) {
    unsigned r;
    asm("v_pk_ashrrev_i16 %0, %1, %2" : "=v"(r) : "v"(fifteen), "v"(v));
    return r;
}
__device__ __forceinline__ unsigned bfi(unsigned mask, unsigned a, unsigned b) {
    unsigned r;
    asm("v_bfi_b32 %0, %1, %2, %3" : "=v"(r) : "s"(mask), "v"(a), "v"(b));
    return r;
}
__device__ __forceinline__ unsigned bfi_v(unsigned mask, unsigned a, unsigned b) {
    unsigned r;
    asm("v_bfi_b32 %0, %1, %2, %3" : "=v"(r) : "v"(mask), "v"(a), "v"(b));
    return r;
}
__device__ __forceinline__ unsigned ge_word(unsigned a, unsigned b) { return sub_v(or_k<GUARD>(a), b); }
__device__ __forceinline__ unsigned lt_word(unsigned a, unsigned b) {
    unsigned r;
    asm("v_pk_sub_i16 %0, %1, %2" : "=v"(r) : "v"(a), "v"(b));
    return r;
}
template <unsigned LIT>
__device__ __forceinline__ unsigned lit_minus(unsigned a) {
    unsigned r;
    asm("v_sub_u32_e32 %0, %2, %1" : "=v"(r) : "v"(a), "n"(LIT));
    return r;
}

struct Cell {
    unsigned hmoe, hg, emex, fmex;
};

template <bool FIRST>
__device__ __forceinline__ void dp_cell(Cell &c, unsigned &acc, unsigned prof, unsigned tsh, unsigned e, unsigned eo, unsigned f,
                                        unsigned fo) {
    const unsigned s = and_k<7u * K1>(pk_shr(prof, tsh));
    const unsigned nzn = lit_minus<(CB - OE) * K1 | GUARD>(c.hmoe);
    const unsigned d = add_v(c.hmoe, s);
    const unsigned en = add_k<0u - (unsigned)EX * K1>(e), fn = add_k<0u - (unsigned)EX * K1>(f);
    const unsigned m = pk_max3(d, en, fn);
    const unsigned dwn = lt_word(d, m), ewn = lt_word(en, m);
    c.hmoe = add_k<0u - 4u * K1>(m);
    c.hg = or_k<GUARD>(c.hmoe);
    c.emex = en;
    c.fmex = fn;
    const unsigned lwn = bfi_v(dwn, ewn, nzn);
    const unsigned p1 = (unsigned)__builtin_amdgcn_perm(dwn, lwn, 0x07030501u), p2 = (unsigned)__builtin_amdgcn_perm(eo, fo, 0x07030501u);
    const unsigned n = bfi(0x80808080u, p1, shr_k<1>(p2));
    acc = FIRST ? n : bfi(0xC0C0C0C0u, n, shr_k<2>(acc));
}

struct State {
    Cell A, B, C, D;
    unsigned qb, t0, t1, t2, t3;
    unsigned best, brow;
    unsigned s0[4], s1[4];
};

__device__ __forceinline__ void track_pair(State &s, const unsigned (&h0)[4], const unsigned (&h1)[4], unsigned step_k, unsigned fifteen) {
    const unsigned risen = pk_max3(pk_max3(h0[0], h0[1], h0[2]), pk_max3(h0[3], h1[0], h1[1]), pk_max3(h1[2], h1[3], s.best));
    const unsigned rose = pk_sign_mask(lt_word(s.best, risen), fifteen);
    s.best = risen;
    s.brow = bfi_v(rose, step_k, s.brow);
#pragma unroll
    for (int k = 0; k < 4; ++k) {
        s.s0[k] = bfi_v(rose, h0[k], s.s0[k]);
        s.s1[k] = bfi_v(rose, h1[k], s.s1[k]);
    }
}

template <int P, bool FIRST>
__device__ __forceinline__ void dp_step(State &s, unsigned (&acc)[4], unsigned (&hs)[4], unsigned prof_mine, unsigned t_next,
                                        unsigned first_all, unsigned last_all, unsigned twelve) {
    constexpr bool ROW = P <= 16;
    s.qb = prof_mine;

    const unsigned eA = bfi_v(first_all, twelve, from_lower<ROW>(pk_max3(s.D.hmoe, s.D.emex, twelve)));
    const unsigned eoA = from_lower<ROW>(sub_v(s.D.hg, s.D.emex));
    dp_cell<FIRST>(s.A, acc[0], s.qb, s.t0, eA, eoA, pk_max(s.B.hmoe, s.B.fmex), sub_v(s.B.hg, s.B.fmex));
    dp_cell<FIRST>(s.B, acc[1], s.qb, s.t1, pk_max3(s.A.hmoe, s.A.emex, twelve), sub_v(s.A.hg, s.A.emex),
                   pk_max(s.C.hmoe, s.C.fmex), sub_v(s.C.hg, s.C.fmex));
    dp_cell<FIRST>(s.C, acc[2], s.qb, s.t2, pk_max3(s.B.hmoe, s.B.emex, twelve), sub_v(s.B.hg, s.B.emex),
                   pk_max(s.D.hmoe, s.D.fmex), sub_v(s.D.hg, s.D.fmex));
    const unsigned fD = bfi_v(last_all, twelve, from_upper<ROW>(pk_max(s.A.hmoe, s.A.fmex)));
    const unsigned foD = from_upper<ROW>(sub_v(s.A.hg, s.A.fmex));
    dp_cell<FIRST>(s.D, acc[3], s.qb, s.t3, pk_max3(s.C.hmoe, s.C.emex, twelve), sub_v(s.C.hg, s.C.emex), fD, foD);

    hs[0] = s.A.hmoe; hs[1] = s.B.hmoe; hs[2] = s.C.hmoe; hs[3] = s.D.hmoe;
    s.t0 = s.t1; s.t1 = s.t2; s.t2 = s.t3;
    s.t3 = t_next;
}

constexpr int PROF_WORDS = 16 * (CH + 4);
constexpr int TCODE_HALVES = 16 * (CH + 3 * 4 + 4 + 4);
constexpr int TWORD_WORDS = 2 * 128;
constexpr int SPREAD_WORDS = 256;

template <int P>
__device__ __forceinline__ void sw_class(const KpBatchView &b, const KpGenes &genes, const KpTask *__restrict__ tasks,
                                         uint32_t n_tasks, const uint32_t *__restrict__ order,
                                         KpSwEnd *__restrict__ ends, uint4 *__restrict__ trace,
                                         unsigned long long *__restrict__ trace_top, uint64_t trace_cap, uint32_t block,
                                         uint32_t n_blocks, unsigned int *__restrict__ next_quad, uint32_t *s_prof_raw,
                                         uint16_t *s_t_raw, uint32_t *s_tw_raw, const uint32_t *s_spread) {
    constexpr int G = 64 / P;
    constexpr int TW = CH + 3 * P + 4;
    constexpr int PAD = (4 - (3 * P + 1) % 4) % 4;
    constexpr int TROW = (TW + PAD + 3) & ~3;
    constexpr int PROW = CH + P;
    static_assert(G * PROW <= PROF_WORDS && G * TROW <= TCODE_HALVES, "LDS carve-up");
    uint32_t(*s_prof)[PROW] = reinterpret_cast<uint32_t(*)[PROW]>(s_prof_raw);
    uint16_t(*s_t)[TROW] = reinterpret_cast<uint16_t(*)[TROW]>(s_t_raw);

    const int lane = threadIdx.x;
    const int g = lane / P, l = lane % P;
    unsigned first_all = l == 0 ? ~0u : 0u, last_all = l == P - 1 ? ~0u : 0u;
    unsigned twelve = CB * K1, fifteen = 15u * K1;
    asm volatile("" : "+v"(twelve), "+v"(fifteen), "+v"(first_all), "+v"(last_all));

    auto take = [&]() -> uint32_t {
        uint32_t q = 0;
        if (lane == 0) q = atomicAdd(next_quad, 1u);
        return (uint32_t)__builtin_amdgcn_readfirstlane((int)q);
    };
    for (uint32_t quad = next_quad ? take() : block; (uint64_t)quad * (2 * G) < n_tasks;
         quad = next_quad ? take() : quad + n_blocks) {
        bool have[2];
        uint32_t ti[2];
        KpTask tk[2];
        int qlen[2], lo[2], q0[2], n_runs[2], steps[2], n_chunks[2];
        int32_t cstart[2], cend[2];
        uint32_t asm_n_words[2], q_off[2], w_off[2], run_off[2];
#pragma unroll
        for (int h = 0; h < 2; ++h) {
            const uint32_t slot = (quad * G + g) * 2 + h;
            have[h] = slot < n_tasks;
            ti[h] = have[h] ? order[slot] : 0u;
            tk[h].asm_id = 0; tk[h].gs = 0; tk[h].contig = 0; tk[h].lo = 0;
            if (have[h]) {
                const int4 head = *reinterpret_cast<const int4 *>(&tasks[ti[h]]);
                tk[h].asm_id = head.x; tk[h].gs = head.y; tk[h].contig = head.z; tk[h].lo = head.w;
            }
            const int gene = tk[h].gs >> 1;
            qlen[h] = have[h] ? genes.len[gene] : 0;
            q_off[h] = (uint32_t)genes.word_off[(tk[h].gs & 1) ? genes.n_genes + gene : gene];
            w_off[h] = (uint32_t)b.asm_word_off[tk[h].asm_id];
            asm_n_words[h] = (uint32_t)(b.asm_word_off[tk[h].asm_id + 1] - b.asm_word_off[tk[h].asm_id]);
            const int c_abs = b.asm_first_ctg[tk[h].asm_id] + tk[h].contig;
            cstart[h] = b.ctg_start[c_abs]; cend[h] = cstart[h] + b.ctg_len[c_abs];
            const int r0 = b.asm_first_nrun[tk[h].asm_id];
            n_runs[h] = b.asm_first_nrun[tk[h].asm_id + 1] - r0;
            run_off[h] = 2u * (uint32_t)r0;
            int r_hi;
            kp_task_rows(tk[h].lo, 4 * P, cstart[h], cend[h], qlen[h], &q0[h], &r_hi);
            lo[h] = tk[h].lo + q0[h];
            steps[h] = have[h] ? (r_hi - q0[h]) + P - 1 : 0;
            n_chunks[h] = (((steps[h] + 7) >> 3) + 3) & ~3;
        }
        int max_steps = max(steps[0], steps[1]);
#pragma unroll
        for (int o = 32; o >= 1; o >>= 1) max_steps = max(max_steps, __shfl_xor(max_steps, o));
        const unsigned long long want = (unsigned long long)P * (unsigned)((have[0] ? n_chunks[0] : 0) + (have[1] ? n_chunks[1] : 0));
        const unsigned long long toff = kp_trace_take(trace_top, have[0] && l == 0, want, g * P);
        const bool fits = have[0] && toff + want <= trace_cap;
        const unsigned long long toff_y = toff + (unsigned long long)P * (unsigned)n_chunks[0];
        uint4 *trace_x = trace + toff + TG * l, *trace_y = trace + toff_y + TG * l;

        State st;
        st.A.hmoe = GAP_EDGE; st.A.hg = GAP_EDGE | GUARD; st.A.emex = GAP_NONE; st.A.fmex = GAP_NONE;
        st.B = st.A; st.C = st.A; st.D = st.A;
        st.qb = PROF_OUT; st.t0 = st.t1 = st.t2 = st.t3 = T_OUT * K1;
        st.best = GAP_EDGE; st.brow = 0;
#pragma unroll
        for (int k = 0; k < 4; ++k) st.s0[k] = st.s1[k] = GAP_EDGE;
        unsigned acc[4] = {0, 0, 0, 0}, held[4] = {0, 0, 0, 0};
        bool saw_n[2] = {have[0] && genes.has_n[tk[0].gs >> 1] != 0, have[1] && genes.has_n[tk[1].gs >> 1] != 0};

        const int steps8 = (max_steps + 7) & ~7;
        constexpr int NQ = (CH / 8 + P - 1) / P, NTW = (TROW + 15) / 16 + 1, NT = (NTW + P - 1) / P;
        static_assert(2 * G * NTW <= TWORD_WORDS, "LDS carve-up");
        uint32_t(*s_tw)[G][NTW] = reinterpret_cast<uint32_t(*)[G][NTW]>(s_tw_raw);
        uint4 qreg[2][NQ];
        uint32_t treg[2][NT];
        auto request = [&](int m0) {
#pragma unroll
            for (int h = 0; h < 2; ++h) {
#pragma unroll
                for (int i = 0; i < NQ; ++i) {
                    const int w = l + i * P, r = q0[h] + m0 + 8 * w;
                    qreg[h][i] = (have[h] && w < CH / 8 && r < qlen[h]) ? genes.prof[q_off[h] + (uint32_t)(r >> 3)] : make_uint4(0u, 0u, 0u, 0u);
                }
                const int w0 = (lo[h] + m0 - PAD) >> 4;
#pragma unroll
                for (int i = 0; i < NT; ++i) {
                    const int wi = w0 + l + i * P;
                    treg[h][i] = (have[h] && l + i * P < NTW && wi >= 0 && (uint32_t)wi < asm_n_words[h]) ? b.words[w_off[h] + (uint32_t)wi] : 0u;
                }
            }
        };
        request(0);
        for (int m0 = 0; m0 < steps8; m0 += CH) {
            __syncthreads();
            {
                const uint32_t keep = m0 == 0 ? PROF_OUT : s_prof[g][CH + l];
                s_prof[g][l] = keep;
            }
#pragma unroll
            for (int i = 0; i < NQ; ++i) {
                const int w = l + i * P;
                if (w < CH / 8) {
                    const uint4 x = qreg[0][i], y = qreg[1][i];
                    uint4 *dst = reinterpret_cast<uint4 *>(&s_prof[g][P + 8 * w]);
                    dst[0] = make_uint4(__builtin_amdgcn_perm(y.x, x.x, 0x05040100u), __builtin_amdgcn_perm(y.x, x.x, 0x07060302u),
                                        __builtin_amdgcn_perm(y.y, x.y, 0x05040100u), __builtin_amdgcn_perm(y.y, x.y, 0x07060302u));
                    dst[1] = make_uint4(__builtin_amdgcn_perm(y.z, x.z, 0x05040100u), __builtin_amdgcn_perm(y.z, x.z, 0x07060302u),
                                        __builtin_amdgcn_perm(y.w, x.w, 0x05040100u), __builtin_amdgcn_perm(y.w, x.w, 0x07060302u));
                }
            }
#pragma unroll
            for (int h = 0; h < 2; ++h)
#pragma unroll
                for (int i = 0; i < NT; ++i)
                    if (l + i * P < NTW) s_tw[h][g][l + i * P] = treg[h][i];
            __syncthreads();
            {
                for (int y = 4 * l; y < TROW; y += 4 * P) {
                    uint32_t four[2];
#pragma unroll
                    for (int h = 0; h < 2; ++h) {
                        const int pw = lo[h] + m0 - PAD, w0 = pw >> 4;
                        const int t0 = pw + y;
                        if (have[h] && n_runs[h] == 0 && t0 >= cstart[h] && t0 + 3 < cend[h]) {
                            const int wi = (t0 >> 4) - w0;
                            const uint32_t lo_w = s_tw[h][g][wi], hi_w = wi + 1 < NTW ? s_tw[h][g][wi + 1] : 0u;
                            four[h] = s_spread[__builtin_amdgcn_alignbit(hi_w, lo_w, 2 * (t0 & 15)) & 255u];
                        } else {
                            four[h] = 0;
                            for (int i = 0; i < 4; ++i) {
                                const int t = t0 + i;
                                unsigned code = 5u;
                                if (have[h] && t >= cstart[h] && t < cend[h]) {
                                    code = (s_tw[h][g][(t >> 4) - w0] >> (2 * (t & 15))) & 3u;
                                    if (kp_in_n_run(b.n_runs + run_off[h], n_runs[h], t)) code = 4u;
                                }
                                four[h] |= (code < 5u ? 3u * code : T_OUT) << (8 * i);
                                saw_n[h] |= code == 4u;
                            }
                        }
                    }
                    const uint32_t lo2 = __builtin_amdgcn_perm(four[1], four[0], 0x05010400u);
                    const uint32_t hi2 = __builtin_amdgcn_perm(four[1], four[0], 0x07030602u);
                    *reinterpret_cast<uint2 *>(&s_t[g][y]) = make_uint2(lo2, hi2);
                }
            }
            __syncthreads();
            if (m0 + CH < steps8) request(m0 + CH);
            if (m0 == 0) {
                const unsigned a0 = s_t[g][PAD + 3 * l], a1 = s_t[g][PAD + 3 * l + 1], a2 = s_t[g][PAD + 3 * l + 2],
                               a3 = s_t[g][PAD + 3 * l + 3];
                st.t0 = (a0 & 255u) | ((a0 >> 8) << 16); st.t1 = (a1 & 255u) | ((a1 >> 8) << 16);
                st.t2 = (a2 & 255u) | ((a2 >> 8) << 16); st.t3 = (a3 & 255u) | ((a3 >> 8) << 16);
            }
            const int m_end = min(m0 + CH, steps8);
            for (int m = m0; m < m_end; m += 8) {
#pragma unroll
                for (int half = 0; half < 2; ++half) {
                    const int mm = m + 4 * half;
                    const uint32_t *pp = &s_prof[g][mm - m0 + P - l];
                    const uint16_t *tp = &s_t[g][mm - m0 + 3 * l + 4 + PAD];
                    const unsigned p0 = pp[0], p1 = pp[1], p2 = pp[2], p3 = pp[3];
                    const unsigned c0 = tp[0], c1 = tp[1], c2 = tp[2], c3 = tp[3];
                    const unsigned ta = __builtin_amdgcn_perm(0u, c0, 0x0c010c00u), tb = __builtin_amdgcn_perm(0u, c1, 0x0c010c00u);
                    const unsigned tcw = __builtin_amdgcn_perm(0u, c2, 0x0c010c00u), td = __builtin_amdgcn_perm(0u, c3, 0x0c010c00u);
                    unsigned h0[4], h1[4];
                    dp_step<P, true>(st, acc, h0, p0, ta, first_all, last_all, twelve);
                    dp_step<P, false>(st, acc, h1, p1, tb, first_all, last_all, twelve);
                    track_pair(st, h0, h1, (unsigned)mm * K1, fifteen);
                    dp_step<P, false>(st, acc, h0, p2, tcw, first_all, last_all, twelve);
                    dp_step<P, false>(st, acc, h1, p3, td, first_all, last_all, twelve);
                    track_pair(st, h0, h1, (unsigned)(mm + 2) * K1, fifteen);
                    if (half == 0) {
#pragma unroll
                        for (int c = 0; c < 4; ++c) held[c] = acc[c];
                    }
                }
                const int j = m >> 3;
                if (fits && j < n_chunks[0])
                    trace_x[(size_t)(j / TG) * (TG * P) + (j % TG)] = make_uint4(__builtin_amdgcn_perm(acc[0], held[0], 0x05040100u), __builtin_amdgcn_perm(acc[1], held[1], 0x05040100u),
                                                        __builtin_amdgcn_perm(acc[2], held[2], 0x05040100u), __builtin_amdgcn_perm(acc[3], held[3], 0x05040100u));
                if (fits && have[1] && j < n_chunks[1])
                    trace_y[(size_t)(j / TG) * (TG * P) + (j % TG)] = make_uint4(__builtin_amdgcn_perm(acc[0], held[0], 0x07060302u), __builtin_amdgcn_perm(acc[1], held[1], 0x07060302u),
                                                        __builtin_amdgcn_perm(acc[2], held[2], 0x07060302u), __builtin_amdgcn_perm(acc[3], held[3], 0x07060302u));
            }
        }

#pragma unroll
        for (int h = 0; h < 2; ++h) {
            const unsigned v = (st.best >> (16 * h)) & 0xFFFFu;
            int mstar = (int)((st.brow >> (16 * h)) & 0xFFFFu), cell = 3;
            bool in0 = false;
#pragma unroll
            for (int k = 3; k >= 0; --k)
                if (((st.s0[k] >> (16 * h)) & 0xFFFFu) == v) { cell = k; in0 = true; }
            if (!in0) {
                ++mstar;
#pragma unroll
                for (int k = 2; k >= 0; --k)
                    if (((st.s1[k] >> (16 * h)) & 0xFFFFu) == v) cell = k;
            }
            int eb = 4 * l + cell;
            unsigned key = v > ZB ? ((v - ZB) << 15) | (unsigned)(32767 - (q0[h] + mstar - l)) : 0u;
            if (key == 0u) eb = 4 * l;
            bool sn = saw_n[h];
#pragma unroll
            for (int o = 1; o < P; o <<= 1) {
                const unsigned key2 = (unsigned)__shfl_xor((int)key, o);
                const int eb2 = __shfl_xor(eb, o);
                if (key2 > key || (key2 == key && eb2 < eb)) { key = key2; eb = eb2; }
                sn |= __shfl_xor((int)sn, o) != 0;
            }
            if (have[h] && l == 0) {
                KpSwEnd out;
                out.score = fits ? (int)(key >> 15) : 0;
                out.er = 32767 - (int)(key & 32767u);
                out.eb = eb | (sn ? KP_SWEND_HAS_N : 0);
                out.trace_off = (uint32_t)(h ? toff_y : toff);
                ends[ti[h]] = out;
            }
        }
    }
}

#ifndef KP_SW_WIDE_BLOCKS
#define KP_SW_WIDE_BLOCKS 512
#endif
constexpr uint32_t WIDE_BLOCKS = KP_SW_WIDE_BLOCKS;
#ifndef KP_SW_HELP_BLOCKS
#define KP_SW_HELP_BLOCKS 3072
#endif
constexpr uint32_t HELP_BLOCKS = KP_SW_HELP_BLOCKS;
#ifndef KP_SW_NARROW_BLOCKS_PER_CU
#define KP_SW_NARROW_BLOCKS_PER_CU 32
#endif
constexpr uint32_t NARROW_BLOCKS_PER_CU = KP_SW_NARROW_BLOCKS_PER_CU;

#ifndef KP_SW_WAVES
#define KP_SW_WAVES 3
#endif
#ifndef KP_SW_LDS_PAD
#define KP_SW_LDS_PAD 0
#endif
__global__ __launch_bounds__(64, KP_SW_WAVES) void kp_sw_kernel(KpBatchView b, KpGenes genes, const KpTask *__restrict__ tasks,
                                                   const uint32_t *__restrict__ task_count, uint32_t task_cap,
                                                   const uint32_t *__restrict__ order, KpSwEnd *__restrict__ ends,
                                                   uint4 *__restrict__ trace, unsigned long long *__restrict__ trace_top,
                                                   uint64_t trace_cap) {
    __shared__ __attribute__((aligned(16))) uint32_t s_prof[PROF_WORDS];
    __shared__ __attribute__((aligned(16))) uint16_t s_t[TCODE_HALVES];
    __shared__ uint32_t s_tw[TWORD_WORDS];
    __shared__ uint32_t s_spread[SPREAD_WORDS];
#if KP_SW_LDS_PAD
    __shared__ uint32_t s_pad[KP_SW_LDS_PAD / 4];
    if (task_cap == 0xFFFFFFFFu) { s_pad[threadIdx.x] = blockIdx.x; __syncthreads(); trace_top[3] = s_pad[63 - threadIdx.x]; }
#endif
    for (uint32_t v = threadIdx.x; v < SPREAD_WORDS; v += 64)
        s_spread[v] = 3u * ((v & 3u) | ((v & 0xCu) << 6) | ((v & 0x30u) << 12) | ((v & 0xC0u) << 18));
    const uint32_t blk = blockIdx.x, narrow_end = 3 * WIDE_BLOCKS + 256u * NARROW_BLOCKS_PER_CU;
    const int c = blk < 3 * WIDE_BLOCKS ? 3 - (int)(blk / WIDE_BLOCKS) : blk < narrow_end ? 0 : 3 - (int)((blk - narrow_end) / (HELP_BLOCKS ? HELP_BLOCKS : 1u));
    const size_t off = (size_t)c * task_cap;
    uint32_t n = task_count[c];
    if (n > task_cap) n = task_cap;
    unsigned int *next_quad = reinterpret_cast<unsigned int *>(trace_top + 1) + c;
    if (c == 3) sw_class<32>(b, genes, tasks + off, n, order + off, ends + off, trace, trace_top, trace_cap, 0, 1, next_quad, s_prof, s_t, s_tw, s_spread);
    else if (c == 2) sw_class<16>(b, genes, tasks + off, n, order + off, ends + off, trace, trace_top, trace_cap, 0, 1, next_quad, s_prof, s_t, s_tw, s_spread);
    else if (c == 1) sw_class<8>(b, genes, tasks + off, n, order + off, ends + off, trace, trace_top, trace_cap, 0, 1, next_quad, s_prof, s_t, s_tw, s_spread);
    else sw_class<4>(b, genes, tasks + off, n, order + off, ends + off, trace, trace_top, trace_cap, 0, 1, next_quad, s_prof, s_t, s_tw, s_spread);
}


constexpr int LONG_NEG = -(1 << 29);

template <int P>
__device__ __forceinline__ void sw_long_class(const KpBatchView &b, const KpGenes &genes, const KpTask *__restrict__ tasks,
                                              const uint32_t *__restrict__ order, uint32_t n_tasks, KpSwEnd *__restrict__ ends,
                                              uint4 *__restrict__ trace, unsigned long long *__restrict__ trace_top, uint64_t trace_cap,
                                              uint32_t block, uint32_t n_blocks) {
    constexpr int G = 64 / P;
    const int lane = threadIdx.x, g = lane / P, l = lane % P;
    for (uint32_t quad = block; (uint64_t)quad * G < n_tasks; quad += n_blocks) {
        const uint32_t slot = quad * G + g;
        const bool have = slot < n_tasks;
        const uint32_t ti = have ? order[slot] : 0u;
        KpTask tk;
        tk.asm_id = 0; tk.gs = 0; tk.contig = 0; tk.lo = 0;
        if (have) tk = tasks[ti];
        const KpTaskSeqs s = kp_task_seqs(b, genes, tk.asm_id, tk.gs, tk.contig);
        int q0, r_hi;
        kp_task_rows(tk.lo, 4 * P, s.t.cstart, s.t.cend, have ? s.q.len : 0, &q0, &r_hi);
        const int steps = have ? (r_hi - q0) + P - 1 : 0;
        const int n_chunks = (((steps + 7) >> 3) + 3) & ~3;
        int max_steps = steps;
#pragma unroll
        for (int o = 32; o >= 1; o >>= 1) max_steps = max(max_steps, __shfl_xor(max_steps, o));
        const unsigned long long want = (unsigned long long)P * (unsigned)(have ? n_chunks : 0);
        const unsigned long long toff = kp_trace_take(trace_top, have && l == 0, want, g * P);
        const bool fits = have && toff + want <= trace_cap;
        uint4 *trace_x = trace + toff + TG * l;
        int H[4] = {0, 0, 0, 0}, E[4], F[4], tc[4];
        bool saw_n = have && genes.has_n[tk.gs >> 1] != 0;
#pragma unroll
        for (int k = 0; k < 4; ++k) { E[k] = F[k] = LONG_NEG; tc[k] = 5; }
        int best = 0, best_r = 0, best_b = 4 * l;
        uint32_t word[4] = {0, 0, 0, 0};
        const int steps8 = (max_steps + 7) & ~7;
        for (int m = 0; m < steps8; ++m) {
            const int r = q0 + m - l;
            const bool row_ok = have && r >= q0 && r < r_hi;
            const int qc = row_ok ? s.q.code(r) : 4;
            const int t0 = tk.lo + r + 4 * l;
#pragma unroll
            for (int k = 0; k < 4; ++k) tc[k] = row_ok ? s.t.code(t0 + k) : 5;
            int hl = __shfl_up(H[3], 1), el = __shfl_up(E[3], 1);
            if (l == 0) { hl = 0; el = LONG_NEG; }
            const int oldH[4] = {H[0], H[1], H[2], H[3]}, oldF[4] = {F[0], F[1], F[2], F[3]};
            const int sh = 2 * (m & 3) + 16 * ((m >> 2) & 1);
            int hu_d = 0, fu_d = LONG_NEG;
#pragma unroll
            for (int k = 0; k < 4; ++k) {
                if (k == 3) {
                    hu_d = __shfl_down(H[0], 1); fu_d = __shfl_down(F[0], 1);
                    if (l == P - 1) { hu_d = 0; fu_d = LONG_NEG; }
                }
                const int hleft = k == 0 ? hl : H[k - 1], eleft = k == 0 ? el : E[k - 1];
                const int hup = k == 3 ? hu_d : oldH[k + 1], fup = k == 3 ? fu_d : oldF[k + 1];
                const int hd = oldH[k];
                const int code = tc[k];
                const bool inside = row_ok && code < 5;
                saw_n |= inside && code == 4;
                const int e_open = hleft - OE, e_ext = eleft - EX, f_open = hup - OE, f_ext = fup - EX;
                const int e = e_open >= e_ext ? e_open : e_ext, f = f_open >= f_ext ? f_open : f_ext;
                int bv = hd + kp_sub_score(qc, code), tb = 0;
                if (e > bv) { bv = e; tb = 1; }
                if (f > bv) { bv = f; tb = 2; }
                const uint32_t not_d = tb != 0, not_l = tb == 0 ? (hd == 0) : (tb == 2);
                const uint32_t eo = e_open >= e_ext, fo = f_open >= f_ext;
                word[k] |= ((not_d << 9) | (eo << 8) | (not_l << 1) | fo) << sh;
                if (inside) {
                    E[k] = e; F[k] = f;
                    H[k] = bv > 0 ? bv : 0;
                    if (bv > best) { best = bv; best_r = r; best_b = 4 * l + k; }
                } else {
                    H[k] = 0; E[k] = LONG_NEG; F[k] = LONG_NEG;
                }
            }
            if ((m & 7) == 7) {
                const int j = m >> 3;
                if (fits && j < n_chunks) trace_x[(size_t)(j / TG) * (TG * P) + (j % TG)] = make_uint4(word[0], word[1], word[2], word[3]);
                word[0] = word[1] = word[2] = word[3] = 0;
            }
        }
        kp_group_best<P>(best, best_r, best_b);
        bool sn = saw_n;
#pragma unroll
        for (int o = 1; o < P; o <<= 1) sn |= __shfl_xor((int)sn, o) != 0;
        if (have && l == 0) {
            KpSwEnd out;
            out.score = fits ? best : 0;
            out.er = best > 0 ? best_r : q0;
            out.eb = (best > 0 ? best_b : 0) | (sn ? KP_SWEND_HAS_N : 0);
            out.trace_off = (uint32_t)toff;
            ends[ti] = out;
        }
    }
}

__global__ __launch_bounds__(64) void kp_sw_long_kernel(KpBatchView b, KpGenes genes, const KpTask *__restrict__ tasks,
                                                        const uint32_t *__restrict__ order_counts, uint32_t task_cap,
                                                        const uint32_t *__restrict__ order, KpSwEnd *__restrict__ ends,
                                                        uint4 *__restrict__ trace, unsigned long long *__restrict__ trace_top,
                                                        uint64_t trace_cap) {
    const int c = blockIdx.y;
    const uint32_t first = order_counts[c], n = order_counts[KP_N_CLASSES + c];
    if (n == 0) return;
    const size_t off = (size_t)c * task_cap;
    if (c == 3) sw_long_class<32>(b, genes, tasks + off, order + off + first, n, ends + off, trace, trace_top, trace_cap, blockIdx.x, gridDim.x);
    else if (c == 2) sw_long_class<16>(b, genes, tasks + off, order + off + first, n, ends + off, trace, trace_top, trace_cap, blockIdx.x, gridDim.x);
    else if (c == 1) sw_long_class<8>(b, genes, tasks + off, order + off + first, n, ends + off, trace, trace_top, trace_cap, blockIdx.x, gridDim.x);
    else sw_long_class<4>(b, genes, tasks + off, order + off + first, n, ends + off, trace, trace_top, trace_cap, blockIdx.x, gridDim.x);
}

constexpr int TB_THREADS = 256;

__global__ __launch_bounds__(TB_THREADS) void kp_sw_traceback_kernel(KpBatchView b, KpGenes genes, const KpTask *__restrict__ tasks,
                                                              const uint32_t *__restrict__ task_count, uint32_t task_cap,
                                                              const uint32_t *__restrict__ order,
                                                              const KpSwEnd *__restrict__ ends,
                                                              const uint32_t *__restrict__ trace,
                                                              KpSwResult *__restrict__ results) {
    const int cls = blockIdx.y;
    uint32_t n = task_count[cls] + task_count[KP_N_CLASSES + cls];
    if (n > task_cap) n = task_cap;
    const int P = 4 << cls;
    const uint32_t n_iter = (n + 63u) & ~63u;
    for (uint32_t slot = blockIdx.x * blockDim.x + threadIdx.x; slot < n_iter; slot += gridDim.x * blockDim.x) {
        const bool have = slot < n;
        const uint32_t ti = have ? order[(size_t)cls * task_cap + slot] : 0u;
        const size_t at = (size_t)cls * task_cap + ti;
        KpSwEnd e;
        e.score = 0; e.er = 0; e.eb = 0; e.trace_off = 0;
        if (have) e = ends[at];
        KpSwResult out;
        out.score = e.score; out.q_start = out.q_end = out.t_start = out.t_end = out.matches = out.block_len = 0;
        const bool walking = have && e.score >= KP_MIN_DP_SCORE;
        KpTask tk;
        tk.asm_id = 0; tk.gs = 0; tk.contig = 0; tk.lo = 0;
        if (walking) tk = tasks[at];
        const bool has_n = (e.eb & KP_SWEND_HAS_N) != 0;
        const int eb = e.eb & 255;
        const KpTaskSeqs s = kp_task_seqs(b, genes, tk.asm_id, tk.gs, tk.contig);
        int q0 = 0, r_hi;
        if (walking) kp_task_rows(tk.lo, 4 * P, s.t.cstart, s.t.cend, s.q.len, &q0, &r_hi);
        const uint4 *tw = reinterpret_cast<const uint4 *>(trace) + e.trace_off;
        KpBandPath path;
        KpNoVisit nobody;
        kp_band_walk(walking, tk.lo, P, q0, e.er, eb, has_n, tw, s, path, nobody);
        if (!have) continue;
        if (e.score < KP_MIN_DP_SCORE) { results[at] = out; continue; }
        const int matches = has_n ? path.matches : (e.score + 4 * path.diag + path.gap_cost) / 6;
        out.score = e.score + path.credit;
        out.q_start = path.sr; out.q_end = e.er + 1;
        out.t_start = path.sr + tk.lo + path.sb; out.t_end = e.er + tk.lo + eb + 1;
        out.matches = matches; out.block_len = path.cols;
        results[at] = out;
    }
}

}

void kp_launch_sw(const KpBatchView &b, const KpGenes &genes, const KpTasks &t, const KpTrace &trace, bool has_long_genes, hipStream_t stream, hipEvent_t after_fill) {
    const dim3 grid(3 * WIDE_BLOCKS + 256u * NARROW_BLOCKS_PER_CU + 3 * HELP_BLOCKS), block(64);
    hipLaunchKernelGGL(kp_sw_kernel, grid, block, 0, stream, b, genes, t.tasks, t.order_count, t.cap, t.order, t.ends, trace.units, trace.top, trace.cap);
    if (has_long_genes)
        hipLaunchKernelGGL(kp_sw_long_kernel, dim3(256, KP_N_CLASSES), block, 0, stream, b, genes, t.tasks, t.order_count, t.cap, t.order, t.ends,
                           trace.units, trace.top, trace.cap);
    if (after_fill) (void)hipEventRecord(after_fill, stream);
    hipLaunchKernelGGL(kp_sw_traceback_kernel, dim3(2048, KP_N_CLASSES), dim3(TB_THREADS), 0, stream, b, genes, t.tasks, t.order_count,
                       t.cap, t.order, t.ends, reinterpret_cast<const uint32_t *>(trace.units), t.results);
}
```

kaptive_amd/csrc/kp_walk.h:

```cpp
#pragma once

#include "kp_internal.h"
#include "kp_seqs.h"

#ifndef KP_TRACE_GROUP
#define KP_TRACE_GROUP 2
#endif

enum { KP_COL_M = 0, KP_COL_I = 1, KP_COL_D = 2 };

struct KpNoVisit {
    __device__ __forceinline__ void run(int, int) {}
};

__device__ __forceinline__ KpTaskSeqs kp_task_seqs(const KpBatchView &b, const KpGenes &genes, int asm_id, int gs, int contig) {
    KpTaskSeqs s;
    const int gene = gs >> 1, c_abs = b.asm_first_ctg[asm_id] + contig, r0 = b.asm_first_nrun[asm_id];
    s.q.nib = genes.nib + genes.word_off[(gs & 1) ? genes.n_genes + gene : gene];
    s.q.len = genes.len[gene];
    s.t.words = b.words + b.asm_word_off[asm_id];
    s.t.n_words = (int)(b.asm_word_off[asm_id + 1] - b.asm_word_off[asm_id]);
    s.t.runs = b.n_runs + 2 * (size_t)r0;
    s.t.n_runs = b.asm_first_nrun[asm_id + 1] - r0;
    s.t.cstart = b.ctg_start[c_abs];
    s.t.cend = s.t.cstart + b.ctg_len[c_abs];
    return s;
}

__device__ __forceinline__ unsigned long long kp_trace_take(unsigned long long *trace_top, bool takes, unsigned long long want, int leader) {
    unsigned long long toff = 0;
    if (takes) toff = atomicAdd(trace_top, want);
    return ((unsigned long long)__shfl((unsigned)(toff >> 32), leader) << 32) | __shfl((unsigned)toff, leader);
}
template <int P>
__device__ __forceinline__ void kp_group_best(int &best, int &best_r, int &best_b) {
#pragma unroll
    for (int o = 1; o < P; o <<= 1) {
        const int s2 = __shfl_xor(best, o), r2 = __shfl_xor(best_r, o), b2 = __shfl_xor(best_b, o);
        if (s2 > best || (s2 == best && (r2 < best_r || (r2 == best_r && b2 < best_b)))) { best = s2; best_r = r2; best_b = b2; }
    }
}

__device__ __forceinline__ uint32_t kp_piece_word(const uint4 &v, int k) {
    const uint32_t lo = (k & 1) ? v.y : v.x, hi = (k & 1) ? v.w : v.z;
    return (k & 2) ? hi : lo;
}

struct KpBandPath {
    int sr, sb;
    int cols, matches , diag, gap_cost, credit;
};

template <class V>
__device__ __forceinline__ void kp_band_walk(bool walking, int lo, int P, int q0, int er, int eb, bool has_n, const uint4 *tw,
                                             const KpTaskSeqs &s, KpBandPath &out, V &v) {
    constexpr int TG = KP_TRACE_GROUP;
    constexpr int EX = KP_GAP_EXT;
    int r = er, bi = eb, state = 0, cols = 0, matches = 0, diag = 0, gap_cost = 0, gap = 0, credit = 0;
    int sr = r, sb = bi;
    uint4 curq[TG], nxtq[TG];
#pragma unroll
    for (int i = 0; i < TG; ++i) curq[i] = nxtq[i] = make_uint4(0, 0, 0, 0);
    int cur_tag = -1, nxt_tag = -1;
    while (__any(walking)) {
        if (!walking) continue;
        const int l = bi >> 2, k = bi & 3, step = r - q0 + l;
        const int pc = step >> 3, grp = pc / TG, tag = (l << 20) | grp;
        if (tag != cur_tag) {
            const uint4 *stream = tw + TG * l;
            if (tag == nxt_tag) {
#pragma unroll
                for (int i = 0; i < TG; ++i) curq[i] = nxtq[i];
            } else {
#pragma unroll
                for (int i = 0; i < TG; ++i) curq[i] = stream[(size_t)grp * (TG * P) + i];
            }
            cur_tag = tag;
            if (grp > 0) {
#pragma unroll
                for (int i = 0; i < TG; ++i) nxtq[i] = stream[(size_t)(grp - 1) * (TG * P) + i];
                nxt_tag = tag - 1;
            }
        }
        uint4 cur = (pc & 1) ? curq[1] : curq[0];
        if (TG == 4) {
            const uint4 hi2 = (pc & 1) ? curq[TG - 1] : curq[TG - 2];
            cur = (pc & 2) ? hi2 : cur;
        }
        const uint32_t word = kp_piece_word(cur, k);
        if (state == 0 && !has_n && (step & 7) == 7 && (word & 0xAAAAAAAAu) == 0u) {
            int n = 8;
#ifndef KP_TB_NO16
            if (TG == 2 && (pc & 1) && (kp_piece_word(curq[0], k) & 0xAAAAAAAAu) == 0u) n = 16;
#endif
            cols += n; diag += n; r -= n;
            v.run(KP_COL_M, n);
            continue;
        }
        const uint32_t half = word >> (16 * ((step >> 2) & 1)), sh = 2 * (step & 3);
        const uint32_t de = ((half >> (8 + sh)) & 3u) ^ 2u, lf = ((half >> sh) & 3u) ^ 2u;
        const uint32_t nib = ((de & 2u) << 2) | ((lf & 2u) << 1) | ((de & 1u) << 1) | (lf & 1u);
        const uint32_t src = (nib & 8u) ? ((nib & 4u) ? 0u : 1u) : ((nib & 4u) ? 2u : 3u);
        if (state == 0) {
            if (src <= 1u) {
                ++cols; ++diag;
                v.run(KP_COL_M, 1);
                if (has_n) {
                    const int qc = s.q.code(r), tc = s.t.at(lo + r + bi);
                    matches += (qc == tc && qc < 4) ? 1 : 0;
                }
                if (src == 1u) { sr = r; sb = bi; walking = false; }
                --r;
            } else {
                state = (int)src - 1;
            }
        } else if (state == 1) {
            ++cols; ++gap; gap_cost += EX;
            v.run(KP_COL_D, 1);
            --bi;
            if (nib & 2u) { state = 0; gap_cost += KP_GAP_OPEN; credit += max(gap - KP_GAP_LONG, 0); gap = 0; }
        } else {
            ++cols; ++gap; gap_cost += EX;
            v.run(KP_COL_I, 1);
            --r; ++bi;
            if (nib & 1u) { state = 0; gap_cost += KP_GAP_OPEN; credit += max(gap - KP_GAP_LONG, 0); gap = 0; }
        }
    }
    out.sr = sr; out.sb = sb; out.cols = cols; out.matches = matches; out.diag = diag; out.gap_cost = gap_cost; out.credit = credit;
}

enum { XT_DIAG = 0, XT_E = 1, XT_F = 2, XT_RESTART = 3, XT_X1 = 4, XT_X2 = 5 };

struct KpJoinPath {
    bool rejected;
    int visited;
    int sr, sb, spk;
    int matches, cols, credit, bonus;
};

template <class V>
__device__ __forceinline__ void kp_join_walk(const KpJoin *J, int k, int P, const KpTaskSeqs &s, const uint4 *trace, KpJoinPath &out, V &v) {
    const int W = 4 * P;
    int pk = k, r = J->end_r[k], bi = J->end_b[k], state = 0, matches = 0, cols = 0, gap = 0, credit = 0;
    int sr = r, sb = bi, spk = k, suf = 0, sufmax = 0, gsum = 0, visited = 1 << k, bonus = 0;
    bool rejected = false;
    int lo = J->lo[pk], q0 = 0, r_hi = 0;
    kp_piece_rows(lo, W, s.t.cstart, s.t.cend, s.q.len, J->r0[pk], J->r1[pk], &q0, &r_hi);
    const uint32_t *tr = reinterpret_cast<const uint32_t *>(trace + J->trace_off[pk]);
    for (;;) {
        const int t = r + lo + bi;
        if (state == 0 && (r < q0 || r >= r_hi || bi < 0 || bi >= W || t < s.t.cstart || t >= s.t.cend)) break;
        const uint32_t byte = (tr[(size_t)(r - q0 + (bi >> 2)) * P + (bi >> 2)] >> (8 * (bi & 3))) & 255u;
        if (state == 0) {
            const uint32_t tb = byte & 7u;
            if (tb == XT_RESTART) break;
            if (suf + gsum > sufmax) sufmax = suf + gsum;
            else if ((tb >= XT_X1 || visited != (1 << k)) && sufmax - (suf + gsum) > KP_JOIN_DROP) { rejected = true; break; }
            if (tb == XT_DIAG) {
                sr = r; sb = bi; spk = pk; ++cols;
                v.run(KP_COL_M, 1);
                const int qc = s.q.code(r), tc = s.t.at(t);
                if (qc < 4 && qc == tc) ++matches;
                suf += kp_sub_score(qc, tc);
                --r;
            } else if (tb == XT_E || tb == XT_F) {
                state = (int)tb;
            } else {
                const int lo_prev = J->lo[pk - 1];
                const bool horizontal = lo > lo_prev;
                const unsigned long long *exp = reinterpret_cast<const unsigned long long *>(trace + J->export_off[pk - 1]);
                const int xi = horizontal ? r : t - lo_prev;
                const unsigned long long key = exp[2 * xi + (tb == XT_X1 ? 0 : 1)];
                const int pos = (int)(0xFFFFFFFFu - (uint32_t)key);
                const int ngap = horizontal ? (t - lo_prev) - pos : r - pos;
                cols += ngap;
                v.run(horizontal ? KP_COL_D : KP_COL_I, ngap);
                const int cost = tb == XT_X1 ? KP_GAP_OPEN + KP_GAP_EXT * ngap : KP_GAP_OPEN2 + KP_GAP_EXT2 * ngap;
                suf -= cost; gsum += cost;
                const int lg = KP_GAP_OPEN + kp_log2x2((uint32_t)ngap);
                if (cost > lg) bonus += cost - lg;
                if (horizontal) bi = pos - r;
                else { bi = t - pos - lo_prev; r = pos; }
                --pk; visited |= 1 << pk;
                lo = lo_prev;
                kp_piece_rows(lo, W, s.t.cstart, s.t.cend, s.q.len, J->r0[pk], J->r1[pk], &q0, &r_hi);
                tr = reinterpret_cast<const uint32_t *>(trace + J->trace_off[pk]);
            }
        } else if (state == XT_E) {
            ++cols; ++gap; --bi; suf -= KP_GAP_EXT;
            v.run(KP_COL_D, 1);
            if (!(byte & 8u)) { state = 0; suf -= KP_GAP_OPEN; credit += max(gap - KP_GAP_LONG, 0); gap = 0; }
        } else {
            ++cols; ++gap; --r; ++bi; suf -= KP_GAP_EXT;
            v.run(KP_COL_I, 1);
            if (!(byte & 16u)) { state = 0; suf -= KP_GAP_OPEN; credit += max(gap - KP_GAP_LONG, 0); gap = 0; }
        }
    }
    out.rejected = rejected; out.visited = visited; out.sr = sr; out.sb = sb; out.spk = spk;
    out.matches = matches; out.cols = cols; out.credit = credit; out.bonus = bonus;
}
```

Measured before the change: 45420 assemblies/s.

## Add per-piece plain-diagonal summary bitmaps to skip trace loads in traceback

The SW fill kernels now also write a compact summary word per lane for every 8 trace pieces, with one bit per piece and cell marking whether that piece is all plain diagonal moves. The band walk used by traceback and CIGAR emission reads these summaries to skip long runs of plain diagonal pieces in one step and to prefetch the next non-plain trace group. This removes most trace-buffer loads along long matching diagonals. In exchange the fill kernels do extra packing work and stores, the trace allocation grows slightly, and the walk logic gains complexity. The path is on by default and can be disabled through an environment variable.

```diff
diff --git a/kaptive_amd/csrc/kp_align.hip b/kaptive_amd/csrc/kp_align.hip
--- a/kaptive_amd/csrc/kp_align.hip
+++ b/kaptive_amd/csrc/kp_align.hip
@@ -12,7 +12,7 @@
     kp_launch_join_trace(b->view, ctx->genes, joins, tasks, trace, ctx->opt.join, w->jstream);
     kp_launch_task_order(b->view, ctx->genes, an, tasks, stream);
     KP_HIP_CHECK(ctx, hipEventRecord(w->ev[KP_EV_ORDER], stream));
-    kp_launch_sw(b->view, ctx->genes, tasks, trace, ctx->max_gene_len > KP_FILL16_MAX_GENE_LEN, stream, w->ev[KP_EV_FILL]);
+    kp_launch_sw(b->view, ctx->genes, tasks, trace, ctx->max_gene_len > KP_FILL16_MAX_GENE_LEN, ctx->opt.trace_summary, stream, w->ev[KP_EV_FILL]);
     KP_HIP_CHECK(ctx, hipEventRecord(w->ev[KP_EV_TRACEBACK], stream));
     return KP_OK;
 }
@@ -179,9 +179,9 @@
     KP_HIP_CHECK(ctx, w->d_cig_ops.reserve(w->cigar_cap));
     KP_HIP_CHECK(ctx, hipMemcpyAsync(w->d_cig_hit_off.p, w->hit_off.data(), (n_asm + 1) * sizeof(int64_t), hipMemcpyHostToDevice, ctx->post));
     kp_launch_cigar_locate(b->view, ctx->d_gene_len.p, w->tasks(), w->joins(), w->hits(), w->d_cig_src.p, ctx->post);
-    kp_launch_cigar_walk(b->view, ctx->genes, w->tasks(), w->joins(), w->trace(), w->hits(), w->hit_rows(), w->d_cig_src.p, w->cigars(), false, ctx->post);
+    kp_launch_cigar_walk(b->view, ctx->genes, w->tasks(), w->joins(), w->trace(), w->hits(), w->hit_rows(), w->d_cig_src.p, w->cigars(), false, ctx->opt.trace_summary, ctx->post);
     for (int attempt = 0;; ++attempt) {
-        kp_launch_cigar_walk(b->view, ctx->genes, w->tasks(), w->joins(), w->trace(), w->hits(), w->hit_rows(), w->d_cig_src.p, w->cigars(), true, ctx->post);
+        kp_launch_cigar_walk(b->view, ctx->genes, w->tasks(), w->joins(), w->trace(), w->hits(), w->hit_rows(), w->d_cig_src.p, w->cigars(), true, ctx->opt.trace_summary, ctx->post);
         KP_HIP_CHECK(ctx, hipGetLastError());
         int64_t need = 0;
         if (int frc = fetch_all(ctx, ctx->post, {{&need, w->d_cig_off.p + total, sizeof need}})) return frc;
diff --git a/kaptive_amd/csrc/kp_cigar.hip b/kaptive_amd/csrc/kp_cigar.hip
--- a/kaptive_amd/csrc/kp_cigar.hip
+++ b/kaptive_amd/csrc/kp_cigar.hip
@@ -91,7 +91,7 @@
 __global__ __launch_bounds__(WALK_THREADS) void kp_cigar_walk_kernel(KpBatchView b, KpGenes genes, const KpTask *__restrict__ tasks,
                                                                      const KpSwEnd *__restrict__ ends, uint32_t task_cap,
                                                                      const KpJoin *__restrict__ joins, uint32_t join_cap,
-                                                                     const uint4 *__restrict__ trace, const uint32_t *__restrict__ n_hits,
+                                                                     const uint4 *__restrict__ trace, bool summaries, const uint32_t *__restrict__ n_hits,
                                                                      uint32_t hit_cap, const int64_t *__restrict__ hit_off,
                                                                      const unsigned long long *__restrict__ src, uint32_t *__restrict__ cnt,
                                                                      const int64_t *__restrict__ off, uint32_t *__restrict__ ops, int64_t ops_cap) {
@@ -117,10 +117,10 @@
                 tk = tasks[at]; e = ends[at];
             }
             const KpTaskSeqs s = kp_task_seqs(b, genes, a, is_join ? J->gs : tk.gs, is_join ? J->contig : tk.contig);
-            int q0 = 0, r_hi;
+            int q0 = 0, r_hi = 0;
             if (is_task) kp_task_rows(tk.lo, 4 * P, s.t.cstart, s.t.cend, s.q.len, &q0, &r_hi);
             KpBandPath bp;
-            kp_band_walk(is_task, tk.lo, P, q0, e.er, e.eb & 255, false, trace + e.trace_off, s, bp, v);
+            kp_band_walk(is_task, summaries, tk.lo, P, q0, r_hi, e.er, e.eb & 255, false, trace + e.trace_off, s, bp, v);
             if (is_join) {
                 KpJoinPath jp;
                 kp_join_walk(J, (int)(ref & 7u), P, s, trace, jp, v);
@@ -167,13 +167,13 @@
 }
 
 void kp_launch_cigar_walk(const KpBatchView &b, const KpGenes &genes, const KpTasks &t, const KpJoins &j, const KpTrace &trace, const KpHitTable &hits,
-                          const KpHitRows &rows, const unsigned long long *src, const KpPerHit<uint32_t> &cig, bool emit, hipStream_t stream) {
+                          const KpHitRows &rows, const unsigned long long *src, const KpPerHit<uint32_t> &cig, bool emit, bool walk_summaries, hipStream_t stream) {
     const dim3 grid((unsigned)std::min(std::max(b.n_asm, 1), 4096)), block(WALK_THREADS);
     if (!emit) {
-        hipLaunchKernelGGL(kp_cigar_walk_kernel<false>, grid, block, 0, stream, b, genes, t.tasks, t.ends, t.cap, j.list, j.cap, trace.units, hits.count,
+        hipLaunchKernelGGL(kp_cigar_walk_kernel<false>, grid, block, 0, stream, b, genes, t.tasks, t.ends, t.cap, j.list, j.cap, trace.units, walk_summaries, hits.count,
                            hits.cap, rows.hit_off, src, cig.cnt, (const int64_t *)nullptr, (uint32_t *)nullptr, (int64_t)0);
         return kp_launch_count_scan(cig.cnt, rows.total, cig.off, stream);
     }
-    hipLaunchKernelGGL(kp_cigar_walk_kernel<true>, grid, block, 0, stream, b, genes, t.tasks, t.ends, t.cap, j.list, j.cap, trace.units, hits.count,
+    hipLaunchKernelGGL(kp_cigar_walk_kernel<true>, grid, block, 0, stream, b, genes, t.tasks, t.ends, t.cap, j.list, j.cap, trace.units, walk_summaries, hits.count,
                        hits.cap, rows.hit_off, src, (uint32_t *)nullptr, cig.off, cig.data, cig.cap);
 }
diff --git a/kaptive_amd/csrc/kp_ctx.hip b/kaptive_amd/csrc/kp_ctx.hip
--- a/kaptive_amd/csrc/kp_ctx.hip
+++ b/kaptive_amd/csrc/kp_ctx.hip
@@ -117,6 +117,7 @@
     o.upload_piece_mb = std::max<uint32_t>(1, env_u32("KAPTIVE_AMD_UPLOAD_PIECE_MB", 4096));
     { const char *rb = getenv("KAPTIVE_AMD_READBACK"); o.readback_copy_engine = rb && std::string(rb) == "copy"; }
     o.spin_wait = (int)env_u32("KAPTIVE_AMD_SPIN_WAIT", 0);
+    { const char *ts = std::getenv("KAPTIVE_AMD_TRACE_SUMMARY"); o.trace_summary = !(ts && std::string(ts) == "0"); }
     o.join_stats = std::getenv("KAPTIVE_AMD_JOIN_STATS") != nullptr;
     if (const char *e = std::getenv("KAPTIVE_AMD_JOIN_GRID")) std::sscanf(e, "%d,%d,%d,%d", &o.join.fill, &o.join.walk, &o.join.chain, &o.join.chain_large);
     if (const char *e = std::getenv("KAPTIVE_AMD_JOIN_PRIO")) o.join.prio = std::atoi(e);
diff --git a/kaptive_amd/csrc/kp_host.h b/kaptive_amd/csrc/kp_host.h
--- a/kaptive_amd/csrc/kp_host.h
+++ b/kaptive_amd/csrc/kp_host.h
@@ -63,6 +63,7 @@
     int spin_wait = 0;
     int cigar = 0;
     int cs = 0;
+    bool trace_summary = true;
     bool join_stats = false;
     KpJoinLaunch join;
 };
diff --git a/kaptive_amd/csrc/kp_internal.h b/kaptive_amd/csrc/kp_internal.h
--- a/kaptive_amd/csrc/kp_internal.h
+++ b/kaptive_amd/csrc/kp_internal.h
@@ -220,7 +220,7 @@
 void kp_launch_occ_cut(const KpBatchView &b, const int32_t *gene_len, const KpAnchors &an, uint32_t *occ_keys, uint32_t *occ_cnts,
                        uint32_t *occ_state, unsigned long long *occ_demand, uint32_t occ_slots, uint32_t occ_log2_size, hipStream_t stream);
 void kp_launch_chain(const KpBatchView &b, const KpAnchors &an, const KpTasks &tasks, const KpGroups &groups, hipStream_t stream);
-void kp_launch_sw(const KpBatchView &b, const KpGenes &genes, const KpTasks &tasks, const KpTrace &trace, bool has_long_genes, hipStream_t stream, hipEvent_t after_fill);
+void kp_launch_sw(const KpBatchView &b, const KpGenes &genes, const KpTasks &tasks, const KpTrace &trace, bool has_long_genes, bool walk_summaries, hipStream_t stream, hipEvent_t after_fill);
 #define KP_ORDER_BUCKETS 65
 #define KP_ORDER_COUNTS (2 * KP_N_CLASSES * KP_ORDER_BUCKETS)
 #define KP_ORDER_HEAD (KP_ORDER_COUNTS + 2 * KP_N_CLASSES)
@@ -234,7 +234,7 @@
 void kp_launch_cigar_locate(const KpBatchView &b, const int32_t *gene_len, const KpTasks &tasks, const KpJoins &joins, const KpHitTable &hits,
                             unsigned long long *src, hipStream_t stream);
 void kp_launch_cigar_walk(const KpBatchView &b, const KpGenes &genes, const KpTasks &tasks, const KpJoins &joins, const KpTrace &trace, const KpHitTable &hits,
-                          const KpHitRows &rows, const unsigned long long *src, const KpPerHit<uint32_t> &cig, bool emit, hipStream_t stream);
+                          const KpHitRows &rows, const unsigned long long *src, const KpPerHit<uint32_t> &cig, bool emit, bool walk_summaries, hipStream_t stream);
 void kp_launch_count_scan(const uint32_t *cnt, int64_t n, int64_t *off, hipStream_t stream);
 void kp_launch_cs_walk(const KpBatchView &b, const KpGenes &genes, const KpHitTable &hits, const KpHitRows &rows, const KpPerHit<uint32_t> &cig,
                        const KpPerHit<char> &cs, bool emit, hipStream_t stream);
diff --git a/kaptive_amd/csrc/kp_sw.hip b/kaptive_amd/csrc/kp_sw.hip
--- a/kaptive_amd/csrc/kp_sw.hip
+++ b/kaptive_amd/csrc/kp_sw.hip
@@ -4,7 +4,6 @@
 namespace {
 
 constexpr int CH = 64;
-constexpr int TG = KP_TRACE_GROUP;
 constexpr int OE = KP_GAP_OPEN + KP_GAP_EXT;
 constexpr int EX = KP_GAP_EXT;
 static_assert(KP_SC_MATCH == 2 && KP_SC_MISMATCH == -4 && KP_SC_N == -1 && OE == 6 && EX == 2,
@@ -105,6 +104,16 @@
 __device__ __forceinline__ unsigned bfi_v(unsigned mask, unsigned a, unsigned b) {
     unsigned r;
     asm("v_bfi_b32 %0, %1, %2, %3" : "=v"(r) : "v"(mask), "v"(a), "v"(b));
+    return r;
+}
+__device__ __forceinline__ unsigned pk_min(unsigned a, unsigned b) {
+    unsigned r;
+    asm("v_pk_min_u16 %0, %1, %2" : "=v"(r) : "v"(a), "v"(b));
+    return r;
+}
+__device__ __forceinline__ unsigned shl1_or(unsigned a, unsigned b) {
+    unsigned r;
+    asm("v_lshl_or_b32 %0, %1, 1, %2" : "=v"(r) : "v"(a), "v"(b));
     return r;
 }
 __device__ __forceinline__ unsigned ge_word(unsigned a, unsigned b) { return sub_v(or_k<GUARD>(a), b); }
@@ -208,8 +217,8 @@
     const int lane = threadIdx.x;
     const int g = lane / P, l = lane % P;
     unsigned first_all = l == 0 ? ~0u : 0u, last_all = l == P - 1 ? ~0u : 0u;
-    unsigned twelve = CB * K1, fifteen = 15u * K1;
-    asm volatile("" : "+v"(twelve), "+v"(fifteen), "+v"(first_all), "+v"(last_all));
+    unsigned twelve = CB * K1, fifteen = 15u * K1, one = K1;
+    asm volatile("" : "+v"(twelve), "+v"(fifteen), "+v"(one), "+v"(first_all), "+v"(last_all));
 
     auto take = [&]() -> uint32_t {
         uint32_t q = 0;
@@ -221,7 +230,8 @@
         bool have[2];
         uint32_t ti[2];
         KpTask tk[2];
-        int qlen[2], lo[2], q0[2], n_runs[2], steps[2], n_chunks[2];
+        int qlen[2], lo[2], q0[2], n_runs[2], steps[2];
+        KpTraceBlock tb[2];
         int32_t cstart[2], cend[2];
         uint32_t asm_n_words[2], q_off[2], w_off[2], run_off[2];
 #pragma unroll
@@ -248,16 +258,18 @@
             kp_task_rows(tk[h].lo, 4 * P, cstart[h], cend[h], qlen[h], &q0[h], &r_hi);
             lo[h] = tk[h].lo + q0[h];
             steps[h] = have[h] ? (r_hi - q0[h]) + P - 1 : 0;
-            n_chunks[h] = (((steps[h] + 7) >> 3) + 3) & ~3;
+            tb[h] = kp_trace_block(P, steps[h]);
         }
         int max_steps = max(steps[0], steps[1]);
 #pragma unroll
         for (int o = 32; o >= 1; o >>= 1) max_steps = max(max_steps, __shfl_xor(max_steps, o));
-        const unsigned long long want = (unsigned long long)P * (unsigned)((have[0] ? n_chunks[0] : 0) + (have[1] ? n_chunks[1] : 0));
+        const unsigned long long want = (unsigned long long)tb[0].units() + tb[1].units();
         const unsigned long long toff = kp_trace_take(trace_top, have[0] && l == 0, want, g * P);
         const bool fits = have[0] && toff + want <= trace_cap;
-        const unsigned long long toff_y = toff + (unsigned long long)P * (unsigned)n_chunks[0];
-        uint4 *trace_x = trace + toff + TG * l, *trace_y = trace + toff_y + TG * l;
+        const unsigned long long toff_y = toff + tb[0].units();
+        uint4 *trace_x = trace + toff + tb[0].piece_at(0, l), *trace_y = trace + toff_y + tb[1].piece_at(0, l);
+        const uint32_t sum_dx = 16u * (tb[0].sum_off() - (uint32_t)tb[0].piece_at(0, l)) + 4u * (uint32_t)tb[0].sum_at(0, l);
+        const uint32_t sum_dy = 16u * (tb[1].sum_off() - (uint32_t)tb[1].piece_at(0, l)) + 4u * (uint32_t)tb[1].sum_at(0, l);
 
         State st;
         st.A.hmoe = GAP_EDGE; st.A.hg = GAP_EDGE | GUARD; st.A.emex = GAP_NONE; st.A.fmex = GAP_NONE;
@@ -267,6 +279,7 @@
 #pragma unroll
         for (int k = 0; k < 4; ++k) st.s0[k] = st.s1[k] = GAP_EDGE;
         unsigned acc[4] = {0, 0, 0, 0}, held[4] = {0, 0, 0, 0};
+        unsigned np[4] = {0, 0, 0, 0};
         bool saw_n[2] = {have[0] && genes.has_n[tk[0].gs >> 1] != 0, have[1] && genes.has_n[tk[1].gs >> 1] != 0};
 
         const int steps8 = (max_steps + 7) & ~7;
@@ -378,12 +391,27 @@
                     }
                 }
                 const int j = m >> 3;
-                if (fits && j < n_chunks[0])
-                    trace_x[(size_t)(j / TG) * (TG * P) + (j % TG)] = make_uint4(__builtin_amdgcn_perm(acc[0], held[0], 0x05040100u), __builtin_amdgcn_perm(acc[1], held[1], 0x05040100u),
+#pragma unroll
+                for (int c = 0; c < 4; ++c) np[c] = shl1_or(np[c], pk_min(and_k<KP_PLAIN_MASK>(or_v(held[c], acc[c])), one));
+                if (fits && j < tb[0].pieces)
+                    trace_x[tb[0].piece_at(j, 0)] = make_uint4(__builtin_amdgcn_perm(acc[0], held[0], 0x05040100u), __builtin_amdgcn_perm(acc[1], held[1], 0x05040100u),
                                                         __builtin_amdgcn_perm(acc[2], held[2], 0x05040100u), __builtin_amdgcn_perm(acc[3], held[3], 0x05040100u));
-                if (fits && have[1] && j < n_chunks[1])
-                    trace_y[(size_t)(j / TG) * (TG * P) + (j % TG)] = make_uint4(__builtin_amdgcn_perm(acc[0], held[0], 0x07060302u), __builtin_amdgcn_perm(acc[1], held[1], 0x07060302u),
+                if (fits && have[1] && j < tb[1].pieces)
+                    trace_y[tb[1].piece_at(j, 0)] = make_uint4(__builtin_amdgcn_perm(acc[0], held[0], 0x07060302u), __builtin_amdgcn_perm(acc[1], held[1], 0x07060302u),
                                                         __builtin_amdgcn_perm(acc[2], held[2], 0x07060302u), __builtin_amdgcn_perm(acc[3], held[3], 0x07060302u));
+            }
+            {
+                const int ch = m0 / CH, up = 8 - ((m_end - m0) >> 3);
+                const unsigned sx = (__builtin_amdgcn_perm(np[1], np[0], 0x0c0c0400u) | __builtin_amdgcn_perm(np[3], np[2], 0x04000c0cu)) << up;
+                const unsigned sy = (__builtin_amdgcn_perm(np[1], np[0], 0x0c0c0602u) | __builtin_amdgcn_perm(np[3], np[2], 0x06020c0cu)) << up;
+                const uint32_t at = (uint32_t)tb[0].sum_at(ch, 0) * 4u;
+#ifdef KP_SW_NO_SUMMARY_STORE
+                asm volatile("" ::"v"(sx), "v"(sy), "v"(at));
+#else
+                if (fits && 8 * ch < tb[0].pieces) *reinterpret_cast<uint32_t *>(reinterpret_cast<char *>(trace_x) + (sum_dx + at)) = sx;
+                if (fits && have[1] && 8 * ch < tb[1].pieces) *reinterpret_cast<uint32_t *>(reinterpret_cast<char *>(trace_y) + (sum_dy + at)) = sy;
+#endif
+                np[0] = np[1] = np[2] = np[3] = 0;
             }
         }
 
@@ -491,14 +519,16 @@
         int q0, r_hi;
         kp_task_rows(tk.lo, 4 * P, s.t.cstart, s.t.cend, have ? s.q.len : 0, &q0, &r_hi);
         const int steps = have ? (r_hi - q0) + P - 1 : 0;
-        const int n_chunks = (((steps + 7) >> 3) + 3) & ~3;
+        const KpTraceBlock tb = kp_trace_block(P, steps);
         int max_steps = steps;
 #pragma unroll
         for (int o = 32; o >= 1; o >>= 1) max_steps = max(max_steps, __shfl_xor(max_steps, o));
-        const unsigned long long want = (unsigned long long)P * (unsigned)(have ? n_chunks : 0);
+        const unsigned long long want = tb.units();
         const unsigned long long toff = kp_trace_take(trace_top, have && l == 0, want, g * P);
         const bool fits = have && toff + want <= trace_cap;
-        uint4 *trace_x = trace + toff + TG * l;
+        uint4 *trace_x = trace + toff;
+        uint32_t *sum_x = reinterpret_cast<uint32_t *>(trace + toff + tb.sum_off());
+        uint32_t sum = 0;
         int H[4] = {0, 0, 0, 0}, E[4], F[4], tc[4];
         bool saw_n = have && genes.has_n[tk.gs >> 1] != 0;
 #pragma unroll
@@ -548,7 +578,13 @@
             }
             if ((m & 7) == 7) {
                 const int j = m >> 3;
-                if (fits && j < n_chunks) trace_x[(size_t)(j / TG) * (TG * P) + (j % TG)] = make_uint4(word[0], word[1], word[2], word[3]);
+                if (fits && j < tb.pieces) trace_x[tb.piece_at(j, l)] = make_uint4(word[0], word[1], word[2], word[3]);
+#pragma unroll
+                for (int k = 0; k < 4; ++k) sum |= (word[k] & KP_PLAIN_MASK) ? 1u << kp_sum_bit(k, j) : 0u;
+                if ((j & 7) == 7 || m + 1 == steps8) {
+                    if (fits && (j >> 3) < tb.sum_words) sum_x[tb.sum_at(j >> 3, l)] = sum;
+                    sum = 0;
+                }
                 word[0] = word[1] = word[2] = word[3] = 0;
             }
         }
@@ -588,7 +624,7 @@
                                                               const uint32_t *__restrict__ task_count, uint32_t task_cap,
                                                               const uint32_t *__restrict__ order,
                                                               const KpSwEnd *__restrict__ ends,
-                                                              const uint32_t *__restrict__ trace,
+                                                              const uint32_t *__restrict__ trace, bool summaries,
                                                               KpSwResult *__restrict__ results) {
     const int cls = blockIdx.y;
     uint32_t n = task_count[cls] + task_count[KP_N_CLASSES + cls];
@@ -611,12 +647,12 @@
         const bool has_n = (e.eb & KP_SWEND_HAS_N) != 0;
         const int eb = e.eb & 255;
         const KpTaskSeqs s = kp_task_seqs(b, genes, tk.asm_id, tk.gs, tk.contig);
-        int q0 = 0, r_hi;
+        int q0 = 0, r_hi = 0;
         if (walking) kp_task_rows(tk.lo, 4 * P, s.t.cstart, s.t.cend, s.q.len, &q0, &r_hi);
         const uint4 *tw = reinterpret_cast<const uint4 *>(trace) + e.trace_off;
         KpBandPath path;
         KpNoVisit nobody;
-        kp_band_walk(walking, tk.lo, P, q0, e.er, eb, has_n, tw, s, path, nobody);
+        kp_band_walk(walking, summaries, tk.lo, P, q0, r_hi, e.er, eb, has_n, tw, s, path, nobody);
         if (!have) continue;
         if (e.score < KP_MIN_DP_SCORE) { results[at] = out; continue; }
         const int matches = has_n ? path.matches : (e.score + 4 * path.diag + path.gap_cost) / 6;
@@ -630,7 +666,7 @@
 
 }
 
-void kp_launch_sw(const KpBatchView &b, const KpGenes &genes, const KpTasks &t, const KpTrace &trace, bool has_long_genes, hipStream_t stream, hipEvent_t after_fill) {
+void kp_launch_sw(const KpBatchView &b, const KpGenes &genes, const KpTasks &t, const KpTrace &trace, bool has_long_genes, bool walk_summaries, hipStream_t stream, hipEvent_t after_fill) {
     const dim3 grid(3 * WIDE_BLOCKS + 256u * NARROW_BLOCKS_PER_CU + 3 * HELP_BLOCKS), block(64);
     hipLaunchKernelGGL(kp_sw_kernel, grid, block, 0, stream, b, genes, t.tasks, t.order_count, t.cap, t.order, t.ends, trace.units, trace.top, trace.cap);
     if (has_long_genes)
@@ -638,5 +674,5 @@
                            trace.units, trace.top, trace.cap);
     if (after_fill) (void)hipEventRecord(after_fill, stream);
     hipLaunchKernelGGL(kp_sw_traceback_kernel, dim3(2048, KP_N_CLASSES), dim3(TB_THREADS), 0, stream, b, genes, t.tasks, t.order_count,
-                       t.cap, t.order, t.ends, reinterpret_cast<const uint32_t *>(trace.units), t.results);
-}
+                       t.cap, t.order, t.ends, reinterpret_cast<const uint32_t *>(trace.units), walk_summaries, t.results);
+}
diff --git a/kaptive_amd/csrc/kp_walk.h b/kaptive_amd/csrc/kp_walk.h
--- a/kaptive_amd/csrc/kp_walk.h
+++ b/kaptive_amd/csrc/kp_walk.h
@@ -46,40 +46,103 @@
     return (k & 2) ? hi : lo;
 }
 
+constexpr uint32_t KP_PLAIN_MASK = 0xAAAAAAAAu;
+constexpr int KP_SUM_PIECES = 8;
+
+struct KpTraceBlock {
+    int P;
+    int pieces;
+    int sum_words;
+    __host__ __device__ uint32_t sum_off() const { return (uint32_t)P * (uint32_t)pieces; }
+    __host__ __device__ uint32_t units() const { return sum_off() + ((((uint32_t)P * (uint32_t)sum_words + 3u) / 4u + 7u) & ~7u); }
+    __host__ __device__ size_t piece_at(int j, int l) const { return (size_t)(j / KP_TRACE_GROUP) * (KP_TRACE_GROUP * P) + KP_TRACE_GROUP * l + j % KP_TRACE_GROUP; }
+    __host__ __device__ size_t sum_at(int chunk, int l) const { return (size_t)chunk * P + l; }
+};
+__host__ __device__ inline KpTraceBlock kp_trace_block(int P, int steps) {
+    KpTraceBlock t;
+    t.P = P;
+    t.pieces = (((steps + 7) >> 3) + 3) & ~3;
+    t.sum_words = (t.pieces + KP_SUM_PIECES - 1) / KP_SUM_PIECES;
+    return t;
+}
+__host__ __device__ inline int kp_sum_bit(int cell, int piece) { return 8 * cell + 7 - (piece & 7); }
+
 struct KpBandPath {
     int sr, sb;
     int cols, matches , diag, gap_cost, credit;
 };
 
 template <class V>
-__device__ __forceinline__ void kp_band_walk(bool walking, int lo, int P, int q0, int er, int eb, bool has_n, const uint4 *tw,
-                                             const KpTaskSeqs &s, KpBandPath &out, V &v) {
+__device__ __forceinline__ void kp_band_walk(bool walking, bool summaries, int lo, int P, int q0, int r_hi, int er, int eb, bool has_n,
+                                             const uint4 *tw, const KpTaskSeqs &s, KpBandPath &out, V &v) {
     constexpr int TG = KP_TRACE_GROUP;
     constexpr int EX = KP_GAP_EXT;
+    static_assert(KP_SUM_PIECES % TG == 0, "a group of pieces lies in one summary word");
+    const KpTraceBlock blk = kp_trace_block(P, walking ? r_hi - q0 + P - 1 : 0);
+    const uint32_t *sum = reinterpret_cast<const uint32_t *>(tw + blk.sum_off());
     int r = er, bi = eb, state = 0, cols = 0, matches = 0, diag = 0, gap_cost = 0, gap = 0, credit = 0;
     int sr = r, sb = bi;
     uint4 curq[TG], nxtq[TG];
 #pragma unroll
     for (int i = 0; i < TG; ++i) curq[i] = nxtq[i] = make_uint4(0, 0, 0, 0);
     int cur_tag = -1, nxt_tag = -1;
+    uint32_t s_cur = ~0u, s_low = ~0u;
+    int s_tag = -1;
+    auto plain_run = [&](int k, int pc, bool &known) -> int {
+        const int p = pc & 7;
+        const uint32_t hi = ((s_cur >> (8 * k)) & 255u) >> (7 - p);
+        int n = __ffs((int)(hi | (1u << (p + 1)))) - 1;
+        known = n <= p;
+        if (!known) {
+            const int m = __ffs((int)(((s_low >> (8 * k)) & 255u) | 256u)) - 1;
+            n += m;
+            known = m < 8;
+        }
+        return n;
+    };
     while (__any(walking)) {
         if (!walking) continue;
         const int l = bi >> 2, k = bi & 3, step = r - q0 + l;
         const int pc = step >> 3, grp = pc / TG, tag = (l << 20) | grp;
+        if (summaries) {
+            const int ch = pc / KP_SUM_PIECES, stag = (l << 20) | ch;
+            if (stag != s_tag) {
+                s_cur = stag + 1 == s_tag && (s_tag & 0xFFFFF) != 0 ? s_low : sum[blk.sum_at(ch, l)];
+                s_low = ch > 0 ? sum[blk.sum_at(ch - 1, l)] : ~0u;
+                s_tag = stag;
+            }
+            if (state == 0 && !has_n && (step & 7) == 7) {
+                bool known;
+                const int n = min(plain_run(k, pc, known), pc);
+                if (n > 0) {
+                    cols += 8 * n; diag += 8 * n; r -= 8 * n;
+                    v.run(KP_COL_M, 8 * n);
+                    continue;
+                }
+            }
+        }
         if (tag != cur_tag) {
-            const uint4 *stream = tw + TG * l;
             if (tag == nxt_tag) {
 #pragma unroll
                 for (int i = 0; i < TG; ++i) curq[i] = nxtq[i];
             } else {
 #pragma unroll
-                for (int i = 0; i < TG; ++i) curq[i] = stream[(size_t)grp * (TG * P) + i];
+                for (int i = 0; i < TG; ++i) curq[i] = tw[blk.piece_at(grp * TG, l) + i];
             }
             cur_tag = tag;
-            if (grp > 0) {
-#pragma unroll
-                for (int i = 0; i < TG; ++i) nxtq[i] = stream[(size_t)(grp - 1) * (TG * P) + i];
-                nxt_tag = tag - 1;
+            int ahead = grp - 1;
+            if (summaries && !has_n && grp > 0) {
+                bool known;
+                const int first = grp * TG;
+                int n;
+                if (first & 7) n = plain_run(k, first - 1, known);
+                else { n = __ffs((int)(((s_low >> (8 * k)) & 255u) | 256u)) - 1; known = n < 8; }
+                ahead = known && first - 1 - n >= 0 ? (first - 1 - n) / TG : -1;
+            }
+            if (ahead >= 0) {
+#pragma unroll
+                for (int i = 0; i < TG; ++i) nxtq[i] = tw[blk.piece_at(ahead * TG, l) + i];
+                nxt_tag = (l << 20) | ahead;
             }
         }
         uint4 cur = (pc & 1) ? curq[1] : curq[0];
@@ -88,13 +151,9 @@
             cur = (pc & 2) ? hi2 : cur;
         }
         const uint32_t word = kp_piece_word(cur, k);
-        if (state == 0 && !has_n && (step & 7) == 7 && (word & 0xAAAAAAAAu) == 0u) {
-            int n = 8;
-#ifndef KP_TB_NO16
-            if (TG == 2 && (pc & 1) && (kp_piece_word(curq[0], k) & 0xAAAAAAAAu) == 0u) n = 16;
-#endif
-            cols += n; diag += n; r -= n;
-            v.run(KP_COL_M, n);
+        if (!summaries && state == 0 && !has_n && (step & 7) == 7 && (word & KP_PLAIN_MASK) == 0u) {
+            cols += 8; diag += 8; r -= 8;
+            v.run(KP_COL_M, 8);
             continue;
         }
         const uint32_t half = word >> (16 * ((step >> 2) & 1)), sh = 2 * (step & 3);
```

Result: faster. 46910 assemblies/s, median of 6 (+3.3%).
